# Advanced-Vision-and-Learning-Lab/sparse-view-3dgs-pack

Measured on AMD Instinct MI355X. Metric: train-step views/s (fwd+bwd) @1M Gaussians 1080p, higher is better.
Workload: dtype f32

## Files before the change

### include/gsplat.h

```cpp
#ifndef GSPLAT_H_INCLUDED
#define GSPLAT_H_INCLUDED

#include <stddef.h>
#include <stdint.h>

#ifdef __cplusplus
extern "C" {
#endif

#define GS_ABI_VERSION 7

#define GS_OK 0
#define GS_E_NULL (-1)
#define GS_E_SHAPE (-2)
#define GS_E_SCRATCH (-3)
#define GS_E_OVERFLOW (-4)
#define GS_E_UNSUPPORTED (-5)

#define GS_TILE_X 16
#define GS_TILE_Y 16
#define GS_NUM_CHANNELS 3

typedef struct GsView {
  int32_t image_height;
// ... 129 lines not shown
  void* phase1_done;
  float* extra;
  float* extra_m;
  float* extra_v;
  float* gain;
  float* gain_m;
  float* gain_v;
  float lr_extra, lr_gain;
  int32_t step_extra, step_gain;
  float* grad_out_extra;
  float* grad_out_gain;
  uint8_t* grad_mask;
  uint8_t* dormant;
  int32_t sparse;
  float* grad_out_rest;
} GsStepState;
#define GS_STEP_BLOCK 256
int gs_backward_step(const GsView* view, const GsGaussians* g, const int32_t* radii,
                     const GsScratch* scratch, int64_t num_rendered, const float* dL_dcolor,
                     const float* dL_dinvdepth, const GsStepState* st, void* workspace,
                     size_t workspace_bytes, void* stream);
int gs_backward_step_x(const GsView* view, const GsGaussians* g, const int32_t* radii,
                       const GsScratch* scratch, int64_t num_rendered, const float* dL_dcolor,
                       const float* dL_dinvdepth, const float* dL_dextra_img, const GsStepState* st,
                       void* workspace, size_t workspace_bytes, void* stream);

int gs_step_uninstanced(const GsView* view, const GsGaussians* g, const int32_t* radii,
                        const GsScratch* scratch, const GsStepState* st, void* stream);

int gs_backward_from_rows(const GsView* view, const GsGaussians* g, const int32_t* radii,
                          const GsScratch* scratch, const double* rows, int32_t depth_mode,
                          const GsGrads* grads, void* workspace, size_t workspace_bytes, void* stream);

int gs_export_tile_order(const GsScratch* scratch, int32_t W, int32_t H, uint32_t* out, void* stream);

size_t gs_tile_depth_limit_floats(int32_t W, int32_t H);
int gs_export_tile_stop_depth(const GsScratch* scratch, int32_t W, int32_t H, float* out, void* stream);
#define GS_STATUS_CHECK(tag, num_rendered, overflow, trunc_failed) \
  ((((uint32_t)(tag)) * 2654435761u) ^ (((uint32_t)(num_rendered)) * 40503u) ^ (((uint32_t)(overflow)) << 30) ^ \
   (((uint32_t)(trunc_failed)) << 31) ^ 0x5bd1e995u)
int gs_forward_status(const GsScratch* scratch, uint32_t* out , void* stream);
int gs_forward_tile_order(const GsView* view, const GsScratch* scratch, void* stream);
int gs_debug_blend_stats(const GsScratch* scratch, int32_t P, int32_t W, int32_t H, uint64_t* out, void* stream);
int gs_export_binning_region(const GsScratch* scratch, int32_t W, int32_t H, int64_t num_rendered, uint64_t* keys_sorted,
                             uint32_t* point_list, void* stream);

size_t gs_knn_tmp_bytes(int32_t P);
int gs_knn_mean_dist2(const float* xyz , int32_t P, float* out , void* tmp,
                      size_t tmp_bytes, void* stream);
int gs_knn_mean_dist2_idx(const float* xyz , int32_t P, float* out ,
                          int32_t* nearest , void* tmp, size_t tmp_bytes, void* stream);

size_t gs_grid_encode_tmp_bytes(int64_t B, int32_t D, int32_t L, int32_t C, int64_t n_slots);
int gs_grid_encode_fwd(const float* inputs, int64_t B, int32_t D, const float* embeddings, int64_t n_slots, int32_t C,
                       const int32_t* offsets, int32_t L, float S, int32_t H, int32_t gridtype, int32_t align_corners,
                       int32_t interp, float* outputs, float* dy_dx, void* stream);
int gs_grid_encode_bwd(const float* grad, const float* inputs, int64_t B, int32_t D, int64_t n_slots, int32_t C,
                       const int32_t* offsets, int32_t L, float S, int32_t H, int32_t gridtype, int32_t align_corners,
                       int32_t interp, const float* dy_dx, float* grad_embeddings, float* grad_inputs, void* tmp,
                       size_t tmp_bytes, void* stream);
int gs_sh_encode_fwd(const float* inputs, int64_t B, int32_t degree, float* outputs, void* stream);
int gs_sh_encode_bwd(const float* grad, const float* inputs, int64_t B, int32_t degree, float* grad_inputs, void* stream);


int gs_l1_fwd(const float* a, const float* b, int64_t n, float* sum, void* stream);
int gs_l1_bwd(const float* a, const float* b, int64_t n, float coef, float* grad_a,
              int32_t accumulate, void* stream);

int gs_dwt_haar_fwd(const float* x, int32_t NC, int32_t H, int32_t W, float* ll, float* lh,
                    float* hl, float* hh, void* stream);
int gs_dwt_haar_bwd(const float* dll, const float* dlh, const float* dhl, const float* dhh,
                    int32_t NC, int32_t H, int32_t W, float* dx, void* stream);

int gs_dwt2_l1_fwd(const float* pred, const float* gt, int32_t C, int32_t H, int32_t W,
                   float* band_sums, void* stream);
int gs_dwt2_l1_bwd(const float* pred, const float* gt, int32_t C, int32_t H, int32_t W,
                   const float* coef_dev, float* grad_pred, int32_t accumulate, void* stream);

int gs_elf_map(const float* img, int32_t C, int32_t H, int32_t W, float* elf_low ,
               float* elf , void* stream);
int gs_patch_means(const float* elf, int32_t H, int32_t W, int32_t patch, float* means,
                   void* stream);
int gs_patch_dwt_fwd(const float* pred, const float* gt, int32_t C, int32_t H, int32_t W,
                     int32_t patch, const uint8_t* mask, float* sums, void* stream);
int gs_patch_dwt_bwd(const float* pred, const float* gt, int32_t C, int32_t H, int32_t W,
                     int32_t patch, const uint8_t* mask, const float* coef_dev ,
                     float* grad_pred, int32_t accumulate, void* stream);

int gs_ssim_fwd(const float* img1, const float* img2, int32_t B, int32_t C, int32_t H, int32_t W,
                float C1, float C2, float* ssim_map, float* dm_dmu1, float* dm_dsigma1_sq,
                float* dm_dsigma12, void* stream);
int gs_ssim_bwd(const float* img1, const float* img2, int32_t B, int32_t C, int32_t H, int32_t W,
                float C1, float C2, const float* dL_dmap, const float* dm_dmu1,
                const float* dm_dsigma1_sq, const float* dm_dsigma12, float* dL_dimg1,
                void* stream);

int gs_l1_bwd_dev(const float* a, const float* b, int64_t n, const float* coef_dev , float* grad_a,
                  int32_t accumulate, void* stream);
int gs_l1_dwt2_fwd(const float* pred, const float* gt, int32_t C, int32_t H, int32_t W, float* l1_sum,
                   float* band_sums, void* stream);
int gs_l1_dwt2_fwd_clamp(const float* raw, const float* gt, int32_t C, int32_t H, int32_t W, float* l1_sum,
                         float* band_sums, float* clamped_out, void* stream);
int gs_l1_dwt2_patch_fwd_clamp(const float* raw, const float* gt, int32_t C, int32_t H, int32_t W, int32_t ps,
                               const uint8_t* mask, float* l1_sum, float* band_sums, float* patch_sums,
                               float* clamped_out, void* stream);
int gs_l1_dwt2_patch_bwd(const float* pred, const float* gt, int32_t C, int32_t H, int32_t W, int32_t ps,
                         const uint8_t* mask, const float* l1_coef_dev , const float* coef_dev ,
                         const float* patch_coef_dev , float* grad_pred, int32_t accumulate, void* stream);
int gs_l1_dwt2_bwd(const float* pred, const float* gt, int32_t C, int32_t H, int32_t W,
                   const float* l1_coef_dev , const float* coef_dev , float* grad_pred,
                   int32_t accumulate, void* stream);
int64_t gs_dwt_partials_count(int32_t C, int32_t H, int32_t W);
int gs_l1_dwt2_patch_fwd_clamp_p(const float* raw, const float* gt, int32_t C, int32_t H, int32_t W, int32_t ps,
                                 const uint8_t* mask, float* partials, float* clamped_out, void* stream);
int64_t gs_l1_partials_count(int64_t n);
int gs_l1_fwd_p(const float* a, const float* b, int64_t n, float* partials, void* stream);
int64_t gs_depth_l1_partials_count(int64_t n);
int gs_depth_l1(const float* invdepth, const float* mono_invdepth, const float* mask, int64_t n, float* partials, float coef,
                const float* coef_dev, float* grad, void* stream);
int gs_ssim_fwd_sum(const float* img1, const float* img2, int32_t B, int32_t C, int32_t H, int32_t W, float C1,
                    float C2, float* sum_out, float* dm_dmu1, float* dm_dsigma1_sq, float* dm_dsigma12,
                    void* stream);
int64_t gs_ssim_partials_count(int32_t B, int32_t C, int32_t H, int32_t W);
int gs_ssim_fwd_partials(const float* img1, const float* img2, int32_t B, int32_t C, int32_t H, int32_t W, float C1,
                         float C2, float* partials, float* dm_dmu1, float* dm_dsigma1_sq, float* dm_dsigma12,
                         void* stream);
int gs_ssim_bwd_uniform(const float* img1, const float* img2, int32_t B, int32_t C, int32_t H, int32_t W,
                        const float* coef_dev, const float* dm_dmu1, const float* dm_dsigma1_sq,
                        const float* dm_dsigma12, float* dL_dimg1, int32_t accumulate, const float* clamp_src,
                        void* stream);
typedef struct GsLgdwtParams {
  float lambda_dssim;
  float n_pix;
  float n_band1, n_band2;
  float dwt_w[8];
  float patch_w[3];
  float patch_weight;
  float patch_elems_per_sel;
  int32_t dwt_enable, patch_enable;
  int32_t reset_sums;
  int32_t custom_base;
  float w_l1, w_ssim;
} GsLgdwtParams;
int gs_lgdwt_combine(const float* sums, float* running_mean, const GsLgdwtParams* params , float* out,
                     void* stream);
int gs_lgdwt_combine_p(const float* sums, const float* ssim_partials, int64_t n_partials, float* running_mean,
                       const GsLgdwtParams* params , float* out, void* stream);
int gs_lgdwt_combine_pp(const float* sums, const float* ssim_partials, int64_t n_partials, const float* dwt_partials,
                        int64_t n_dwt, const float* l1_partials, int64_t n_l1, float* running_mean,
                        const GsLgdwtParams* params , float* out, void* stream);
int gs_lgdwt_fused_fwd(const float* raw, const float* gt, int32_t C, int32_t H, int32_t W, float C1, float C2, int32_t ps,
                       const uint8_t* mask, float* dwt_partials, float* ssim_partials, float* dm_dmu1, float* dm_dsigma1_sq,
                       float* dm_dsigma12, void* stream);
int gs_lgdwt_fused_bwd(const float* raw, const float* gt, int32_t C, int32_t H, int32_t W, int32_t flags, int32_t ps,
                       const uint8_t* mask, const float* coef_dev, const float* dm_dmu1, const float* dm_dsigma1_sq,
                       const float* dm_dsigma12, float* grad, void* stream);

typedef struct GsAdamSeg {
  int64_t begin, end;
  float lr_a, lr_b;
  int32_t period, split;
  int32_t step;
  int32_t row_width;
} GsAdamSeg;
int gs_adam_step(float* params, const float* grads, float* exp_avg, float* exp_avg_sq, int64_t n,
                 const GsAdamSeg* segs, int32_t nseg, float beta1, float beta2, float eps, int32_t step,
                 void* stream);
int gs_adam_step_gated(float* params, const float* grads, float* exp_avg, float* exp_avg_sq, int64_t n,
                       const GsAdamSeg* segs, int32_t nseg, float beta1, float beta2, float eps, int32_t step,
                       const float* gate, void* stream);
int gs_adam_step_masked(float* params, const float* grads, float* exp_avg, float* exp_avg_sq, int64_t n,
                        const GsAdamSeg* segs, int32_t nseg, float beta1, float beta2, float eps, int32_t step,
                        const float* gate, const float* row_mask, void* stream);

int gs_activations_fwd(const float* scaling , const float* rotation ,
                       const float* opacity , int32_t P, float* scales_out, float* rotations_out,
                       float* opacities_out, void* stream);
int gs_activations_bwd(const float* scaling, const float* rotation, const float* opacity, int32_t P,
                       const float* dL_dscales, const float* dL_drotations, const float* dL_dopacities,
                       float* d_scaling, float* d_rotation, float* d_opacity, void* stream);
int gs_densify_stats(const int32_t* radii, const float* dL_dmeans2D , int32_t P,
                     float* max_radii2D , float* xyz_gradient_accum , float* denom ,
                     void* stream);

int gs_rows_pack(const float* flat, int32_t P, int32_t nfields, const int32_t* widths , const uint8_t* mask,
                 const int32_t* pos, int32_t K, float* packed, void* stream);
int gs_rows_unpack(float* flat, int32_t P, int32_t nfields, const int32_t* widths , const uint8_t* mask,
                   const int32_t* pos, int32_t K, const float* packed, void* stream);
int64_t gs_image_stage_partials_count(int32_t H, int32_t W);
int gs_image_stage_fwd(const float* raw, const float* exposure, const float* alpha, int32_t H, int32_t W, float* pred,
                       void* stream);
int gs_image_stage_bwd(const float* raw, const float* exposure, const float* alpha, const float* g_pred, int32_t H, int32_t W,
                       float* g_raw, float* partials, void* stream);
int gs_exposure_adam(const float* partials, int64_t n_partials, int32_t camera, float* grad, float* exposure, float* exp_avg,
                     float* exp_avg_sq, int32_t n_cameras, float lr, double beta1, double beta2, float eps, int32_t step,
                     const float* gate, void* stream);
int gs_export_row_mask(const GsScratch* scratch, int32_t P, uint8_t* mask, void* stream);

int gs_profile_enable(int32_t on);
int gs_profile_only(int32_t stage);
int gs_profile_reset(void);
int gs_profile_stage_count(void);
const char* gs_profile_stage_name(int32_t stage);
int gs_profile_read(double* ms, int64_t* counts, int32_t n);

#ifdef __cplusplus
}
#endif
#endif
```

### profiles/summarize.py

```python
#!/usr/bin/env python3
import collections
import csv
import glob
import json
import os
import sys

src, tag = sys.argv[1], sys.argv[2]
script_dir = os.path.dirname(os.path.abspath(__file__))
here = sys.argv[3] if len(sys.argv) > 3 else script_dir
sys.path.insert(0, script_dir)
from source_id import source_id


def run_identity():
    ident = {"tag": tag, "source_id": source_id(os.path.dirname(script_dir))}
    try:
        line = [x for x in open(os.path.join(src, "bench_trace.json")).read().splitlines() if x.startswith("{")][-1]
        j = json.loads(line)
        ident["P"] = j["config"]["gaussians"]
        ident["R"] = j["config"]["num_rendered_last_view"]
        ident["workload"] = j["config"]["workload"]
    except Exception as e:
        ident["identity_error"] = repr(e)
    return ident
OURS = ("preprocess_fwd_kernel", "scan_block_sums_kernel", "rs_hist_kernel", "rs_scatter_kernel", "scan_reduce_kernel",
        "scan_sums_kernel", "scan_down_kernel", "rs_rowscan_kernel", "sorted_block_sums_kernel", "duplicate_kernel", "tile_ranges_kernel",
        "bin_prepare_kernel", "render_fwd_wave_kernel", "render_bwd_wave_kernel", "render_fwd_kernel", "render_bwd_kernel", "adam_kernel", "scan_small_kernel", "preprocess_bwd_kernel", "l1_fwd_kernel",
        "l1_bwd_kernel", "dwt2_l1_fwd_kernel", "dwt2_l1_bwd_kernel", "ssim_fwd_kernel", "ssim_bwd_kernel",
        "patch_dwt_kernel", "lgdwt_combine_kernel", "act_fwd_kernel", "act_bwd_kernel", "densify_stats_kernel", "patch_means_kernel", "elf_low_kernel", "bilinear_up_kernel", "knn_search_kernel", "preprocess_bwd_step_kernel",
        "tile_order_kernel", "zero_rows_kernel", "stop_depth_bounds_kernel", "region_bin_kernel", "region_prepare_kernel",
        "status_tag_kernel", "rs_small_sort_kernel", "step_uninstanced_kernel", "chain_kernel",
        "tb_entries_kernel", "tb_emit_kernel", "tb_regions_from_counts_kernel", "tb_regions_kernel", "tb_tile_count_kernel",
        "tb_region_scan_kernel", "tb_tile_scan_kernel", "tb_write_kernel", "depth_l1_kernel", "rows_pack_kernel", "row_mask_kernel",
        "ssim_fwd_clamp_kernel", "lgdwt_bwd_kernel", "lgdwt_fwd_kernel")


def short(name):
    for o in sorted(OURS, key=len, reverse=True):
        if o in name:
            return o
    return name.split("(")[0][-60:]


stats = glob.glob(os.path.join(src, "trace", "*", "*_kernel_stats.csv"))[0]
rows = list(csv.DictReader(open(stats)))
import shutil
shutil.copyfile(stats, os.path.join(here, "%s_rocprofv3_kernel_stats_full.csv" % tag))
with open(os.path.join(here, "%s_kernel_stats.csv" % tag), "w") as f:
    w = csv.writer(f)
    w.writerow(["Name", "Calls", "TotalDurationNs", "AverageNs", "Percentage", "MinNs", "MaxNs"])
    for r in rows[:40]:
        w.writerow([short(r["Name"]), r["Calls"], r["TotalDurationNs"], r["AverageNs"], r["Percentage"], r["MinNs"], r["MaxNs"]])

trace = glob.glob(os.path.join(src, "trace", "*", "*_kernel_trace.csv"))[0]
tr = sorted(csv.DictReader(open(trace)), key=lambda r: int(r["Start_Timestamp"]))
idx = [i for i, r in enumerate(tr) if "render_bwd_wave_kernel" in r["Kernel_Name"] or "render_bwd_kernel" in r["Kernel_Name"]]
a, b = idx[-3], idx[-2]
for j in range(len(idx) - 2, 0, -1):
    if any("step_uninstanced_kernel" in r["Kernel_Name"] for r in tr[idx[j - 1]:idx[j]]):
        a, b = idx[j - 1], idx[j]
        break
seg = tr[a:b]
wall = (int(tr[b]["Start_Timestamp"]) - int(seg[0]["Start_Timestamp"])) / 1e6
t_end = int(tr[b]["Start_Timestamp"])
iv = sorted((int(r["Start_Timestamp"]), min(int(r["End_Timestamp"]), t_end)) for r in seg)
busy, cur_s, cur_e = 0.0, None, None
for s0, e0 in iv:
    if cur_e is None or s0 > cur_e:
        if cur_e is not None:
            busy += cur_e - cur_s
        cur_s, cur_e = s0, e0
    else:
        cur_e = max(cur_e, e0)
busy = (busy + (cur_e - cur_s if cur_e is not None else 0)) / 1e6
agg = collections.OrderedDict()
for r in seg:
    n = short(r["Kernel_Name"])
    agg.setdefault(n, [0.0, 0])
    agg[n][0] += (int(r["End_Timestamp"]) - int(r["Start_Timestamp"])) / 1e3
    agg[n][1] += 1
with open(os.path.join(here, "%s_step_timeline.txt" % tag), "w") as f:
    f.write("one steady-state train step (render_bwd to render_bwd), rocprofv3 --kernel-trace\n")
    f.write("wall %.3f ms, GPU busy %.3f ms, %d kernel launches\n" % (wall, busy, len(seg)))
    for n, (d, c) in sorted(agg.items(), key=lambda x: -x[1][0]):
        f.write("%10.1f us %4d  %s\n" % (d, c, n))

traffic = {}
table = collections.defaultdict(lambda: {"FETCH_SIZE": [], "WRITE_SIZE": []})
for kind in ("fetch", "write"):
    files = glob.glob(os.path.join(src, kind, "*", "*_counter_collection.csv"))
    if not files:
        continue
    for r in csv.DictReader(open(files[0])):
        table[short(r["Kernel_Name"])][r["Counter_Name"]].append(float(r["Counter_Value"]))
with open(os.path.join(here, "%s_pmc_traffic.csv" % tag), "w") as f:
    w = csv.writer(f)
    w.writerow(["kernel", "launches", "FETCH_SIZE_KiB_mean", "WRITE_SIZE_KiB_mean", "hbm_read_bytes_corrected(x2)",
                "hbm_write_bytes", "hbm_total_bytes_per_launch"])
    for k, v in sorted(table.items()):
        if k not in OURS or not v["FETCH_SIZE"]:
            continue
        fs = v["FETCH_SIZE"][-max(1, len(v["FETCH_SIZE"]) // 3):]
        ws = v["WRITE_SIZE"][-max(1, len(v["WRITE_SIZE"]) // 3):] if v["WRITE_SIZE"] else [0.0]
        fm, wm = sum(fs) / len(fs), sum(ws) / len(ws)
        rd, wr = 2.0 * fm * 1024.0, wm * 1024.0
        w.writerow([k, len(v["FETCH_SIZE"]), "%.1f" % fm, "%.1f" % wm, "%.0f" % rd, "%.0f" % wr, "%.0f" % (rd + wr)])
        traffic[k] = rd + wr
stage_of = {"render_bwd": "render_bwd_wave_kernel", "render_fwd": "render_fwd_wave_kernel", "preprocess_fwd": "preprocess_fwd_kernel",
            "preprocess_bwd": "preprocess_bwd_kernel", "preprocess_bwd_step": "preprocess_bwd_step_kernel",
            "duplicate": "duplicate_kernel", "tile_ranges": "tile_ranges_kernel", "region_bin": "region_bin_kernel",
            "ssim_fwd": "ssim_fwd_kernel", "ssim_bwd": "ssim_bwd_kernel",
            "step_uninstanced": "step_uninstanced_kernel", "chain": "chain_kernel"}
for st, kn in (("ssim_fwd", "ssim_fwd_clamp_kernel"), ("ssim_fwd", "lgdwt_fwd_kernel"), ("ssim_bwd", "lgdwt_bwd_kernel")):
    if kn in traffic:
        stage_of[st] = kn
out = {st: traffic[k] for st, k in stage_of.items() if k in traffic}
out.update(run_identity())
out["launches_counted"] = {st: len(table[k]["FETCH_SIZE"]) for st, k in stage_of.items() if k in traffic}
if "region_bin_kernel" in traffic:
    out["sort"] = traffic["region_bin_kernel"]
elif "rs_scatter_kernel" in traffic:
    out["sort"] = 6 * (traffic.get("rs_scatter_kernel", 0) + traffic.get("rs_hist_kernel", 0))
json.dump(out, open(os.path.join(here, "pmc_traffic.json"), "w"), indent=1)
print(open(os.path.join(here, "%s_step_timeline.txt" % tag)).read())
print(open(os.path.join(here, "%s_pmc_traffic.csv" % tag)).read())

sq = collections.defaultdict(lambda: collections.defaultdict(list))
for f in glob.glob(os.path.join(src, "sq[0-9]*", "*", "*_counter_collection.csv")):
    for r in csv.DictReader(open(f)):
        sq[short(r["Kernel_Name"])][r["Counter_Name"]].append(float(r["Counter_Value"]))
if sq:
    with open(os.path.join(here, "%s_sq_counters.csv" % tag), "w") as f:
        w = csv.writer(f)
        w.writerow(["kernel", "waves", "VALU_insts_per_wave", "LDS_insts_per_wave", "SALU_insts_per_wave", "VMEM_rd_per_wave",
                    "VMEM_wr_per_wave", "VALU_issue_pct_of_peak", "VALU_active_x4_pct_of_SIMD_cycles", "wait_any_pct_of_wave_cycles",
                    "wait_inst_pct_of_wave_cycles", "waves_per_SIMD", "LDS_bank_conflict_pct_of_LDS_cycles"])
        sq_insts = run_identity()
        sq_insts["launches_counted"] = {}
        for k, v in sorted(sq.items()):
            m = {c: sum(x) / len(x) for c, x in v.items()}
            if k not in OURS or "GRBM_GUI_ACTIVE" not in m or m.get("SQ_WAVES", 0) == 0:
                continue
            simd_cycles = m["GRBM_GUI_ACTIVE"] / 8 * 1024
            wc = max(1.0, m.get("SQ_WAVE_CYCLES", 0))
            w.writerow([k, int(m["SQ_WAVES"]), round(m.get("SQ_INSTS_VALU", 0) / m["SQ_WAVES"], 1),
                        round(m.get("SQ_INSTS_LDS", 0) / m["SQ_WAVES"], 1), round(m.get("SQ_INSTS_SALU", 0) / m["SQ_WAVES"], 1),
                        round(m.get("SQ_INSTS_VMEM_RD", 0) / m["SQ_WAVES"], 1), round(m.get("SQ_INSTS_VMEM_WR", 0) / m["SQ_WAVES"], 1),
                        round(100 * m.get("SQ_INSTS_VALU", 0) * 2 / simd_cycles, 1),
                        round(100 * m.get("SQ_ACTIVE_INST_VALU", 0) * 4 / simd_cycles, 1),
                        round(100 * m.get("SQ_WAIT_ANY", 0) / wc, 1), round(100 * m.get("SQ_WAIT_INST_ANY", 0) / wc, 1),
                        round(wc * 4 / simd_cycles, 2),
                        round(100 * m.get("SQ_LDS_BANK_CONFLICT", 0) / max(1.0, m.get("SQ_LDS_IDX_ACTIVE", 0)), 1)])
            for st, kn in (("render_bwd", "render_bwd_wave_kernel"), ("render_fwd", "render_fwd_wave_kernel")):
                if k == kn:
                    sq_insts[st] = m.get("SQ_INSTS_VALU", 0)
                    sq_insts["launches_counted"][st] = len(v.get("SQ_INSTS_VALU", []))
                    sq_insts[st + "_valu_active_cycles_per_simd"] = m.get("SQ_ACTIVE_INST_VALU", 0) * 4 / 1024
                    sq_insts[st + "_valu_active_share_under_profiler"] = m.get("SQ_ACTIVE_INST_VALU", 0) * 4 / simd_cycles
    json.dump(sq_insts, open(os.path.join(here, "sq_insts.json"), "w"), indent=1)
    print(open(os.path.join(here, "%s_sq_counters.csv" % tag)).read())


for kind in ("init_like",):
    st_files = glob.glob(os.path.join(src, "trace_" + kind, "*", "*_kernel_stats.csv"))
    if not st_files:
        continue
    shutil.copyfile(st_files[0], os.path.join(here, "%s_%s_rocprofv3_kernel_stats_full.csv" % (tag, kind)))
    with open(os.path.join(here, "%s_%s_kernel_stats.csv" % (tag, kind)), "w") as f:
        w = csv.writer(f)
        w.writerow(["Name", "Calls", "TotalDurationNs", "AverageNs", "Percentage", "MinNs", "MaxNs"])
        for r in list(csv.DictReader(open(st_files[0])))[:30]:
            w.writerow([short(r["Name"]), r["Calls"], r["TotalDurationNs"], r["AverageNs"], r["Percentage"], r["MinNs"], r["MaxNs"]])
    ident = {"tag": tag, "source_id": source_id(os.path.dirname(script_dir)), "scene": kind}
    try:
        line = [x for x in open(os.path.join(src, "bench_trace_%s.json" % kind)).read().splitlines() if x.startswith("{")][-1]
        j = json.loads(line)
        ident["P"], ident["R"] = j["config"]["gaussians"], j["config"]["num_rendered_last_view"]
        shutil.copyfile(os.path.join(src, "bench_trace_%s.json" % kind), os.path.join(here, "%s_%s_bench_under_rocprof.json" % (tag, kind)))
    except Exception as e:
        ident["identity_error"] = repr(e)
    sqk = collections.defaultdict(lambda: collections.defaultdict(list))
    for f in glob.glob(os.path.join(src, "sq_" + kind, "*", "*_counter_collection.csv")):
        for r in csv.DictReader(open(f)):
            sqk[short(r["Kernel_Name"])][r["Counter_Name"]].append(float(r["Counter_Value"]))
    ident["launches_counted"] = {}
    for stn, kn in (("render_bwd", "render_bwd_wave_kernel"), ("render_fwd", "render_fwd_wave_kernel")):
        v = sqk.get(kn, {}).get("SQ_INSTS_VALU", [])
        if v:
            ident[stn] = sum(v) / len(v)
            ident["launches_counted"][stn] = len(v)
            wv = sqk[kn].get("SQ_WAVES", [])
            sa = sqk[kn].get("SQ_INSTS_SALU", [])
            if wv and sum(wv):
                ident[stn + "_valu_per_wave"] = sum(v) / sum(wv) * len(wv) / len(v)
                if sa:
                    ident[stn + "_salu_per_wave"] = sum(sa) / sum(wv) * len(wv) / len(sa)
    json.dump(ident, open(os.path.join(here, "sq_insts_%s.json" % kind), "w"), indent=1)
    print(kind, json.dumps(ident))


st_files = glob.glob(os.path.join(src, "trace_binning", "*", "*_kernel_stats.csv"))
if st_files:
    BIN = ("tb_", "rs_", "scan_sums_kernel", "scan_block_sums_kernel", "bin_prepare_kernel", "preprocess_fwd_kernel", "render_fwd_wave_kernel")
    with open(os.path.join(here, "%s_binning_kernel_stats.csv" % tag), "w") as f:
        w = csv.writer(f)
        w.writerow(["Name", "Calls", "TotalDurationNs", "AverageNs", "MinNs", "MaxNs"])
        for r in csv.DictReader(open(st_files[0])):
            if any(b in r["Name"] for b in BIN):
                w.writerow([r["Name"].split("(")[0][-48:], r["Calls"], r["TotalDurationNs"], r["AverageNs"], r["MinNs"], r["MaxNs"]])
    try:
        shutil.copyfile(os.path.join(src, "binning_trace.log"), os.path.join(here, "%s_binning_probe.log" % tag))
    except OSError:
        pass
    cnt = collections.defaultdict(lambda: collections.defaultdict(list))
    for d_ in ("sq_binning", "fetch_binning", "write_binning"):
        for f in glob.glob(os.path.join(src, d_, "*", "*_counter_collection.csv")):
            for r in csv.DictReader(open(f)):
                cnt[r["Kernel_Name"].split("(")[0][-48:]][r["Counter_Name"]].append(float(r["Counter_Value"]))
    with open(os.path.join(here, "%s_binning_counters.csv" % tag), "w") as f:
        w = csv.writer(f)
        w.writerow(["kernel", "launches", "hbm_read_bytes_corrected(x2)", "hbm_write_bytes", "LDS_insts_per_wave",
                    "LDS_bank_conflict_pct_of_LDS_cycles"])
        for k, v in sorted(cnt.items()):
            if not any(b in k for b in BIN):
                continue
            last = lambda x: x[-max(1, len(x) // 2):]
            m = {c: sum(last(x)) / len(last(x)) for c, x in v.items()}
            w.writerow([k, len(next(iter(v.values()))), "%.0f" % (2048.0 * m.get("FETCH_SIZE", 0)), "%.0f" % (1024.0 * m.get("WRITE_SIZE", 0)),
                        round(m.get("SQ_INSTS_LDS", 0) / max(1.0, m.get("SQ_WAVES", 0)), 1),
                        round(100 * m.get("SQ_LDS_BANK_CONFLICT", 0) / max(1.0, m.get("SQ_LDS_IDX_ACTIVE", 0)), 1)])
    print(open(os.path.join(here, "%s_binning_counters.csv" % tag)).read())
```

### sparse-view-3dgs-pack_amd/csrc/gs_loss.hip

```cpp
#include <cstdlib>

#include "gs_common.h"
#include "gs_prof.h"

#define HC 0.7071067811865476f

struct Bands {
  float ll, lh, hl, hh;
};
__device__ __forceinline__ Bands haar_block(float a, float b, float c, float d) {
  const float lo_t = HC * a + HC * b, hi_t = HC * a - HC * b;
  const float lo_b = HC * c + HC * d, hi_b = HC * c - HC * d;
  Bands r;
  r.ll = HC * lo_t + HC * lo_b;
  r.lh = HC * lo_t - HC * lo_b;
  r.hl = HC * hi_t + HC * hi_b;
  r.hh = HC * hi_t - HC * hi_b;
  return r;
}
__device__ __forceinline__ void haar_block_adj(float gll, float glh, float ghl, float ghh, float& da, float& db,
                                               float& dc, float& dd) {
  const float dlo_t = HC * gll + HC * glh, dlo_b = HC * gll - HC * glh;
  const float dhi_t = HC * ghl + HC * ghh, dhi_b = HC * ghl - HC * ghh;
  da = HC * dlo_t + HC * dhi_t;
// ... 22 lines not shown
  }
}

__global__ void __launch_bounds__(GS_BLOCK) l1_fwd_kernel(const float* __restrict__ a, const float* __restrict__ b,
                                                          int64_t n, float* sum, float* __restrict__ partials) {
  float acc[1] = {0.f};
  const int64_t n4 = n >> 2;
  const float4* a4 = reinterpret_cast<const float4*>(a);
  const float4* b4 = reinterpret_cast<const float4*>(b);
  for (int64_t i = (int64_t)blockIdx.x * GS_BLOCK + threadIdx.x; i < n4; i += (int64_t)gridDim.x * GS_BLOCK) {
    const float4 x = a4[i], y = b4[i];
    acc[0] += fabsf(x.x - y.x) + fabsf(x.y - y.y) + fabsf(x.z - y.z) + fabsf(x.w - y.w);
  }
  if (blockIdx.x == 0 && threadIdx.x < (n & 3)) acc[0] += fabsf(a[n4 * 4 + threadIdx.x] - b[n4 * 4 + threadIdx.x]);
  if (partials) {
    __shared__ float red[GS_BLOCK / 64];
    float x = acc[0];
#pragma unroll
    for (int off = 32; off >= 1; off >>= 1) x += __shfl_down(x, off, 64);
    if ((threadIdx.x & 63) == 0) red[threadIdx.x >> 6] = x;
    __syncthreads();
    if (threadIdx.x == 0) {
      float t = 0.f;
      for (int w = 0; w < GS_BLOCK / 64; w++) t += red[w];
      partials[blockIdx.x] = t;
    }
    return;
  }
  block_sum_atomic<1>(acc, sum);
}
__global__ void __launch_bounds__(GS_BLOCK) l1_bwd_kernel(const float* __restrict__ a, const float* __restrict__ b,
                                                          int64_t n, float coef, const float* __restrict__ coef_dev,
                                                          float* __restrict__ g, int accumulate) {
  if (coef_dev) coef *= coef_dev[0];
  for (int64_t i = (int64_t)blockIdx.x * GS_BLOCK + threadIdx.x; i < n; i += (int64_t)gridDim.x * GS_BLOCK) {
    const float v = coef * sgnf(a[i] - b[i]);
    g[i] = accumulate ? g[i] + v : v;
  }
}

__global__ void __launch_bounds__(GS_BLOCK) depth_l1_kernel(const float* __restrict__ d, const float* __restrict__ m,
                                                            const float* __restrict__ k, int64_t n, float* __restrict__ partials,
                                                            float coef, const float* __restrict__ coef_dev,
                                                            float* __restrict__ grad) {
  if (coef_dev) coef *= coef_dev[0];
  float acc = 0.f;
  for (int64_t i = (int64_t)blockIdx.x * GS_BLOCK + threadIdx.x; i < n; i += (int64_t)gridDim.x * GS_BLOCK) {
    const float w = k ? k[i] : 1.0f;
    const float v = (d[i] - m[i]) * w;
    acc += fabsf(v);
    if (grad) grad[i] = coef * sgnf(v) * w;
  }
  if (partials) {
    __shared__ float red[GS_BLOCK / 64];
#pragma unroll
    for (int off = 32; off >= 1; off >>= 1) acc += __shfl_down(acc, off, 64);
    if ((threadIdx.x & 63) == 0) red[threadIdx.x >> 6] = acc;
    __syncthreads();
    if (threadIdx.x == 0) {
      float t = 0.f;
      for (int w = 0; w < GS_BLOCK / 64; w++) t += red[w];
      partials[blockIdx.x] = t;
    }
  }
}

__global__ void __launch_bounds__(GS_BLOCK) dwt_fwd_kernel(const float* __restrict__ x, int NC, int H, int W, float* ll,
                                                           float* lh, float* hl, float* hh) {
  const int h = cdiv2(H), w = cdiv2(W);
  const int64_t total = (int64_t)NC * h * w;
  for (int64_t o = (int64_t)blockIdx.x * GS_BLOCK + threadIdx.x; o < total; o += (int64_t)gridDim.x * GS_BLOCK) {
    const int j = (int)(o % w), i = (int)((o / w) % h), c = (int)(o / ((int64_t)w * h));
    const float* p = x + (size_t)c * H * W;
    const int y0 = 2 * i, y1 = min(2 * i + 1, H - 1), x0 = 2 * j, x1 = min(2 * j + 1, W - 1);
    const Bands b = haar_block(p[(size_t)y0 * W + x0], p[(size_t)y0 * W + x1], p[(size_t)y1 * W + x0], p[(size_t)y1 * W + x1]);
    if (ll) ll[o] = b.ll;
    if (lh) lh[o] = b.lh;
    if (hl) hl[o] = b.hl;
    if (hh) hh[o] = b.hh;
  }
}
__global__ void __launch_bounds__(GS_BLOCK) dwt_bwd_kernel(const float* dll, const float* dlh, const float* dhl,
                                                           const float* dhh, int NC, int H, int W, float* __restrict__ dx) {
  const int h = cdiv2(H), w = cdiv2(W);
  const int64_t total = (int64_t)NC * h * w;
  for (int64_t o = (int64_t)blockIdx.x * GS_BLOCK + threadIdx.x; o < total; o += (int64_t)gridDim.x * GS_BLOCK) {
    const int j = (int)(o % w), i = (int)((o / w) % h), c = (int)(o / ((int64_t)w * h));
    float da, db, dc, dd;
    haar_block_adj(dll ? dll[o] : 0.f, dlh ? dlh[o] : 0.f, dhl ? dhl[o] : 0.f, dhh ? dhh[o] : 0.f, da, db, dc, dd);
    float* p = dx + (size_t)c * H * W;
    const int y0 = 2 * i, x0 = 2 * j;
    const bool py = 2 * i + 1 >= H, pxp = 2 * j + 1 >= W;
    if (!py && !pxp) {
      p[(size_t)y0 * W + x0] = da;
      p[(size_t)y0 * W + x0 + 1] = db;
      p[(size_t)(y0 + 1) * W + x0] = dc;
      p[(size_t)(y0 + 1) * W + x0 + 1] = dd;
    } else if (py && !pxp) {
      p[(size_t)y0 * W + x0] = da + dc;
      p[(size_t)y0 * W + x0 + 1] = db + dd;
    } else if (!py && pxp) {
      p[(size_t)y0 * W + x0] = da + db;
      p[(size_t)(y0 + 1) * W + x0] = dc + dd;
    } else {
      p[(size_t)y0 * W + x0] = ((da + db) + dc) + dd;
    }
  }
}

struct Px44 {
  float v[4][4];
};
struct Blk44 {
  float l1[2][2][4];
  float l2[4];
};
template <bool FAST>
__device__ __forceinline__ void load_px44(const float* __restrict__ p, int H, int W, int i2, int j2, int h1, int w1,
                                          Px44& o) {
  if (FAST) {
#pragma unroll
    for (int y = 0; y < 4; y++) {
      const float4 q = reinterpret_cast<const float4*>(p + (size_t)(4 * i2 + y) * W)[j2];
      o.v[y][0] = q.x; o.v[y][1] = q.y; o.v[y][2] = q.z; o.v[y][3] = q.w;
    }
  } else {
#pragma unroll
    for (int r = 0; r < 2; r++)
#pragma unroll
      for (int c = 0; c < 2; c++) {
        const int r1 = min(2 * i2 + r, h1 - 1), c1 = min(2 * j2 + c, w1 - 1);
        const int y0 = 2 * r1, y1 = min(2 * r1 + 1, H - 1), x0 = 2 * c1, x1 = min(2 * c1 + 1, W - 1);
        o.v[2 * r][2 * c] = p[(size_t)y0 * W + x0];
        o.v[2 * r][2 * c + 1] = p[(size_t)y0 * W + x1];
        o.v[2 * r + 1][2 * c] = p[(size_t)y1 * W + x0];
        o.v[2 * r + 1][2 * c + 1] = p[(size_t)y1 * W + x1];
      }
  }
}
__device__ __forceinline__ void bands_of(const Px44& x, Blk44& o) {
  float ll[2][2];
#pragma unroll
  for (int r = 0; r < 2; r++)
#pragma unroll
    for (int c = 0; c < 2; c++) {
      const Bands b = haar_block(x.v[2 * r][2 * c], x.v[2 * r][2 * c + 1], x.v[2 * r + 1][2 * c], x.v[2 * r + 1][2 * c + 1]);
      o.l1[r][c][0] = b.ll; o.l1[r][c][1] = b.lh; o.l1[r][c][2] = b.hl; o.l1[r][c][3] = b.hh;
      ll[r][c] = b.ll;
    }
  const Bands b2 = haar_block(ll[0][0], ll[0][1], ll[1][0], ll[1][1]);
  o.l2[0] = b2.ll; o.l2[1] = b2.lh; o.l2[2] = b2.hl; o.l2[3] = b2.hh;
}

template <bool FAST, bool ROWS>
__device__ __forceinline__ void dwt2_l1_fwd_body(const float* __restrict__ pred, const float* __restrict__ gt, int C, int H,
                                                 int W, float* band_sums, float* l1_sum, float* __restrict__ clamped_out,
                                                 const uint8_t* __restrict__ patch_mask, int ps, float* patch_sums,
                                                 float* __restrict__ partials, int clamp, unsigned wg, unsigned nwg,
                                                 float (*red12)[12]) {
  const int h1 = cdiv2(H), w1 = cdiv2(W), h2 = cdiv2(h1), w2 = cdiv2(w1);
  const int64_t total = (int64_t)C * h2 * w2;
  const int pnx = patch_mask ? W / ps : 0, pny = patch_mask ? H / ps : 0;
  float s[12] = {0, 0, 0, 0, 0, 0, 0, 0, 0, 0, 0, 0};
  for (int64_t o = (int64_t)wg * GS_BLOCK + threadIdx.x; o < total; o += (int64_t)nwg * GS_BLOCK) {
    const int j2 = (int)(o % w2), i2 = (int)((o / w2) % h2), c = (int)(o / ((int64_t)w2 * h2));
    Px44 pa, pb;
    load_px44<FAST>(pred + (size_t)c * H * W, H, W, i2, j2, h1, w1, pa);
    load_px44<FAST>(gt + (size_t)c * H * W, H, W, i2, j2, h1, w1, pb);
    if (FAST && (clamped_out || clamp)) {
#pragma unroll
      for (int y = 0; y < 4; y++) {
#pragma unroll
        for (int x = 0; x < 4; x++) pa.v[y][x] = fminf(fmaxf(pa.v[y][x], 0.f), 1.f);
        if (clamped_out)
          reinterpret_cast<float4*>(clamped_out + (size_t)c * H * W + (size_t)(4 * i2 + y) * W)[j2] =
              make_float4(pa.v[y][0], pa.v[y][1], pa.v[y][2], pa.v[y][3]);
      }
    }
    Blk44 a, b;
    bands_of(pa, a);
    bands_of(pb, b);
    bool in_patch = false;
    if (FAST && patch_mask) {
      const int py = (4 * i2) / ps, px = (4 * j2) / ps;
      in_patch = py < pny && px < pnx && patch_mask[py * pnx + px] != 0;
    }
#pragma unroll
    for (int r = 0; r < 2; r++)
#pragma unroll
      for (int cc = 0; cc < 2; cc++)
        if (FAST || (2 * i2 + r < h1 && 2 * j2 + cc < w1)) {
#pragma unroll
          for (int k = 0; k < 4; k++) {
            const float d = fabsf(a.l1[r][cc][k] - b.l1[r][cc][k]);
            s[k] += d;
            if (FAST && k > 0 && in_patch) s[8 + k] += d;
          }
        }
#pragma unroll
    for (int k = 0; k < 4; k++) s[4 + k] += fabsf(a.l2[k] - b.l2[k]);
    if (ROWS || l1_sum) {
#pragma unroll
      for (int y = 0; y < 4; y++)
#pragma unroll
        for (int x = 0; x < 4; x++)
          if (FAST || (4 * i2 + y < H && 4 * j2 + x < W)) s[8] += fabsf(pa.v[y][x] - pb.v[y][x]);
    }
  }
  if (ROWS || l1_sum) {
#pragma unroll
    for (int k = 0; k < 12; k++) {
      float x = s[k];
#pragma unroll
      for (int off = 32; off >= 1; off >>= 1) x += __shfl_down(x, off, 64);
      if ((threadIdx.x & 63) == 0) red12[threadIdx.x >> 6][k] = x;
    }
    __syncthreads();
    if (threadIdx.x < 12) {
      float t = 0.f;
      for (int w = 0; w < GS_BLOCK / 64; w++) t += red12[w][threadIdx.x];
      if (ROWS || partials)
        partials[(size_t)wg * 12 + threadIdx.x] = t;
      else if (t != 0.f)
        atomicAdd(threadIdx.x < 8 ? &band_sums[threadIdx.x] : (threadIdx.x == 8 ? l1_sum : &patch_sums[threadIdx.x - 9]), t);
    }
  } else {
    float s8[8];
#pragma unroll
    for (int k = 0; k < 8; k++) s8[k] = s[k];
    block_sum_atomic<8>(s8, band_sums);
  }
}
template <bool FAST>
__global__ void __launch_bounds__(GS_BLOCK) dwt2_l1_fwd_kernel(const float* __restrict__ pred, const float* __restrict__ gt,
                                                               int C, int H, int W, float* band_sums, float* l1_sum,
                                                               float* __restrict__ clamped_out,
                                                               const uint8_t* __restrict__ patch_mask, int ps,
                                                               float* patch_sums, float* __restrict__ partials, int clamp) {
  __shared__ float red12[GS_BLOCK / 64][12];
  dwt2_l1_fwd_body<FAST, false>(pred, gt, C, H, W, band_sums, l1_sum, clamped_out, patch_mask, ps, patch_sums, partials, clamp,
                         blockIdx.x, gridDim.x, red12);
}

template <bool FAST>
__global__ void __launch_bounds__(GS_BLOCK) dwt2_l1_bwd_kernel(const float* __restrict__ pred, const float* __restrict__ gt,
                                                               int C, int H, int W, const float* __restrict__ coef,
                                                               const float* __restrict__ l1_coef, float* __restrict__ grad,
                                                               int accumulate, const uint8_t* __restrict__ patch_mask, int ps,
                                                               const float* __restrict__ patch_coef) {
  const int h1 = cdiv2(H), w1 = cdiv2(W), h2 = cdiv2(h1), w2 = cdiv2(w1);
  const int64_t total = (int64_t)C * h2 * w2;
  const int pnx = patch_mask ? W / ps : 0, pny = patch_mask ? H / ps : 0;
  float cfg[8];
#pragma unroll
  for (int k = 0; k < 8; k++) cfg[k] = coef[k];
  float cp[3] = {0.f, 0.f, 0.f};
  if (patch_mask) { cp[0] = patch_coef[0]; cp[1] = patch_coef[1]; cp[2] = patch_coef[2]; }
  const float c1l = l1_coef ? l1_coef[0] : 0.f;
  for (int64_t o = (int64_t)blockIdx.x * GS_BLOCK + threadIdx.x; o < total; o += (int64_t)gridDim.x * GS_BLOCK) {
    const int j2 = (int)(o % w2), i2 = (int)((o / w2) % h2), c = (int)(o / ((int64_t)w2 * h2));
    Px44 pa, pb;
    load_px44<FAST>(pred + (size_t)c * H * W, H, W, i2, j2, h1, w1, pa);
    load_px44<FAST>(gt + (size_t)c * H * W, H, W, i2, j2, h1, w1, pb);
    Blk44 a, b;
    bands_of(pa, a);
    bands_of(pb, b);
    float cf[8];
#pragma unroll
    for (int k = 0; k < 8; k++) cf[k] = cfg[k];
    if (FAST && patch_mask) {
      const int py = (4 * i2) / ps, px = (4 * j2) / ps;
      if (py < pny && px < pnx && patch_mask[py * pnx + px] != 0) {
        cf[1] += cp[0];
        cf[2] += cp[1];
        cf[3] += cp[2];
      }
    }
    float dl[2][2];
    {
      float da, db, dc, dd;
      haar_block_adj(cf[4] * sgnf(a.l2[0] - b.l2[0]), cf[5] * sgnf(a.l2[1] - b.l2[1]), cf[6] * sgnf(a.l2[2] - b.l2[2]),
                     cf[7] * sgnf(a.l2[3] - b.l2[3]), da, db, dc, dd);
      const bool pr = !FAST && 2 * i2 + 1 >= h1, pc = !FAST && 2 * j2 + 1 >= w1;
      dl[0][0] = da; dl[0][1] = db; dl[1][0] = dc; dl[1][1] = dd;
      if (pr && pc) { dl[0][0] = ((da + db) + dc) + dd; }
      else if (pr) { dl[0][0] = da + dc; dl[0][1] = db + dd; }
      else if (pc) { dl[0][0] = da + db; dl[1][0] = dc + dd; }
    }
    float* gp = grad + (size_t)c * H * W;
    float out[4][4];
#pragma unroll
    for (int r = 0; r < 2; r++)
#pragma unroll
      for (int cc = 0; cc < 2; cc++) {
        const int r1 = 2 * i2 + r, c1 = 2 * j2 + cc;
        if (!FAST && (r1 >= h1 || c1 >= w1)) continue;
        float da, db, dc, dd;
        haar_block_adj(cf[0] * sgnf(a.l1[r][cc][0] - b.l1[r][cc][0]) + dl[r][cc], cf[1] * sgnf(a.l1[r][cc][1] - b.l1[r][cc][1]),
                       cf[2] * sgnf(a.l1[r][cc][2] - b.l1[r][cc][2]), cf[3] * sgnf(a.l1[r][cc][3] - b.l1[r][cc][3]), da, db,
                       dc, dd);
        const int y0 = 2 * r1, x0 = 2 * c1;
        const bool py = !FAST && y0 + 1 >= H, pxp = !FAST && x0 + 1 >= W;
        float v00 = da, v01 = db, v10 = dc, v11 = dd;
        if (py && pxp) v00 = ((da + db) + dc) + dd;
        else if (py) { v00 = da + dc; v01 = db + dd; }
        else if (pxp) { v00 = da + db; v10 = dc + dd; }
        v00 += c1l * sgnf(pa.v[2 * r][2 * cc] - pb.v[2 * r][2 * cc]);
        v01 += c1l * sgnf(pa.v[2 * r][2 * cc + 1] - pb.v[2 * r][2 * cc + 1]);
        v10 += c1l * sgnf(pa.v[2 * r + 1][2 * cc] - pb.v[2 * r + 1][2 * cc]);
        v11 += c1l * sgnf(pa.v[2 * r + 1][2 * cc + 1] - pb.v[2 * r + 1][2 * cc + 1]);
        if (FAST) {
          out[2 * r][2 * cc] = v00; out[2 * r][2 * cc + 1] = v01; out[2 * r + 1][2 * cc] = v10; out[2 * r + 1][2 * cc + 1] = v11;
        } else {
          float* q = gp + (size_t)y0 * W + x0;
          if (accumulate) {
            q[0] += v00;
            if (!pxp) q[1] += v01;
            if (!py) { q[W] += v10; if (!pxp) q[W + 1] += v11; }
          } else {
            q[0] = v00;
            if (!pxp) q[1] = v01;
            if (!py) { q[W] = v10; if (!pxp) q[W + 1] = v11; }
          }
        }
      }
    if (FAST) {
#pragma unroll
      for (int y = 0; y < 4; y++) {
        float4* q = reinterpret_cast<float4*>(gp + (size_t)(4 * i2 + y) * W) + j2;
        float4 v = make_float4(out[y][0], out[y][1], out[y][2], out[y][3]);
        if (accumulate) { const float4 old = *q; v.x += old.x; v.y += old.y; v.z += old.z; v.w += old.w; }
        *q = v;
      }
    }
  }
}

__global__ void __launch_bounds__(GS_BLOCK) elf_low_kernel(const float* __restrict__ img, int C, int H, int W,
                                                           float* __restrict__ low) {
  const int h = cdiv2(H), w = cdiv2(W);
  const int o = blockIdx.x * GS_BLOCK + threadIdx.x;
  if (o >= h * w) return;
  const int j = o % w, i = o / w;
  const int y0 = 2 * i, y1 = min(2 * i + 1, H - 1), x0 = 2 * j, x1 = min(2 * j + 1, W - 1);
  float s0 = 0.f, s1 = 0.f, s2 = 0.f, s3 = 0.f;
  for (int c = 0; c < C; c++) {
    const float* p = img + (size_t)c * H * W;
    const Bands b = haar_block(p[(size_t)y0 * W + x0], p[(size_t)y0 * W + x1], p[(size_t)y1 * W + x0], p[(size_t)y1 * W + x1]);
    s0 += fabsf(b.ll); s1 += fabsf(b.lh); s2 += fabsf(b.hl); s3 += fabsf(b.hh);
  }
  const float HF = s1 + s2 + s3;
  low[o] = s0 / (s0 + HF + 1e-8f);
}
__global__ void __launch_bounds__(GS_BLOCK) bilinear_up_kernel(const float* __restrict__ low, int h, int w, int H, int W,
                                                               float* __restrict__ out) {
  const int o = blockIdx.x * GS_BLOCK + threadIdx.x;
  if (o >= H * W) return;
  const int x = o % W, y = o / W;
  const float sh = (float)h / (float)H, sw = (float)w / (float)W;
  float sy = sh * ((float)y + 0.5f) - 0.5f;
  if (sy < 0) sy = 0;
  const int y0 = (int)sy, y1 = y0 + (y0 < h - 1 ? 1 : 0);
  const float ly1 = sy - (float)y0, ly0 = 1.f - ly1;
  float sx = sw * ((float)x + 0.5f) - 0.5f;
  if (sx < 0) sx = 0;
  const int x0 = (int)sx, x1 = x0 + (x0 < w - 1 ? 1 : 0);
  const float lx1 = sx - (float)x0, lx0 = 1.f - lx1;
  out[o] = ly0 * (lx0 * low[(size_t)y0 * w + x0] + lx1 * low[(size_t)y0 * w + x1]) +
           ly1 * (lx0 * low[(size_t)y1 * w + x0] + lx1 * low[(size_t)y1 * w + x1]);
}
__global__ void __launch_bounds__(GS_BLOCK) patch_means_kernel(const float* __restrict__ elf, int H, int W, int ps,
                                                               float* __restrict__ means) {
  const int nx = W / ps;
  const int px = blockIdx.x % nx, py = blockIdx.x / nx;
// ... 93 lines not shown
#pragma unroll
    for (int j = 0; j < 4; j++)
#pragma unroll
      for (int q = 0; q < NQ; q++) acc[rd][j][q] = 0.f;
    if (item < NITEM) {
      const int r = item / (ST / 4), c0 = (item % (ST / 4)) * 4;
#pragma unroll
      for (int e = 0; e < 14; e++) {
        float val[NQ];
        if (FWD) {
          const float a = tile[0][r][c0 + e], b = tile[1][r][c0 + e];
          val[0] = a; val[1] = a * a; val[2] = b; val[3 % NQ] = b * b; val[4 % NQ] = a * b;
        } else {
#pragma unroll
          for (int q = 0; q < NQ; q++) val[q] = tile[q][r][c0 + e];
        }
#pragma unroll
        for (int j = 0; j < 4; j++) {
          const int t = e - j;
          if (t >= 0 && t < 11) {
#pragma unroll
            for (int q = 0; q < NQ; q++) acc[rd][j][q] += GW[t] * val[q];
          }
        }
      }
    }
  }
  __syncthreads();
#pragma unroll
  for (int rd = 0; rd < NR; rd++) {
    const int item = threadIdx.x + rd * GS_BLOCK;
    if (item < NITEM) {
      const int r = item / (ST / 4), c0 = (item % (ST / 4)) * 4;
#pragma unroll
      for (int j = 0; j < 4; j++)
#pragma unroll
        for (int q = 0; q < NQ; q++) hor[q][r][c0 + j] = acc[rd][j][q];
    }
  }
  __syncthreads();
  const int lx = threadIdx.x & 31, r0 = (threadIdx.x >> 5) * 4;
#pragma unroll
  for (int j = 0; j < 4; j++)
#pragma unroll
    for (int q = 0; q < NQ; q++) out[j][q] = 0.f;
#pragma unroll
  for (int e = 0; e < 14; e++) {
    float val[NQ];
#pragma unroll
    for (int q = 0; q < NQ; q++) val[q] = hor[q][r0 + e][lx];
#pragma unroll
    for (int j = 0; j < 4; j++) {
      const int t = e - j;
      if (t >= 0 && t < 11) {
#pragma unroll
        for (int q = 0; q < NQ; q++) out[j][q] += GW[t] * val[q];
      }
    }
  }
}

__device__ __forceinline__ float clamp01(float v) { return fminf(fmaxf(v, 0.f), 1.f); }
__device__ __forceinline__ void ssim_stage_fwd(const float* __restrict__ img1, const float* __restrict__ img2, size_t plane,
                                               int H, int W, int bx, int by, bool clamp1, float (*tile)[SH][SH + 1]) {
  const bool vec = (W & 3) == 0 && ((((uintptr_t)img1) | ((uintptr_t)img2)) & 15) == 0;
  if (vec) {
    constexpr int VPR = 12, NV = SH * VPR, NVI = (NV + GS_BLOCK - 1) / GS_BLOCK;
    float4 a[NVI], b[NVI];
#pragma unroll
    for (int it = 0; it < NVI; it++) {
      const int v = threadIdx.x + it * GS_BLOCK;
      const int r = v / VPR, q = v % VPR;
      const int y = by + r - 5, x4 = bx - 8 + 4 * q;
      a[it] = b[it] = make_float4(0.f, 0.f, 0.f, 0.f);
      if (v < NV && y >= 0 && y < H && x4 >= 0 && x4 + 3 < W) {
        a[it] = *reinterpret_cast<const float4*>(img1 + plane + (size_t)y * W + x4);
        b[it] = *reinterpret_cast<const float4*>(img2 + plane + (size_t)y * W + x4);
      }
    }
#pragma unroll
    for (int it = 0; it < NVI; it++) {
      const int v = threadIdx.x + it * GS_BLOCK;
      if (v < NV) {
        const int r = v / VPR, c0 = 4 * (v % VPR) - 3;
        const float av[4] = {a[it].x, a[it].y, a[it].z, a[it].w}, bv[4] = {b[it].x, b[it].y, b[it].z, b[it].w};
#pragma unroll
        for (int e = 0; e < 4; e++) {
          const int c = c0 + e;
          if (c >= 0 && c < SH) {
            tile[0][r][c] = clamp1 ? clamp01(av[e]) : av[e];
            tile[1][r][c] = bv[e];
          }
        }
      }
    }
  } else {
    constexpr int NIT = (SH * SH + GS_BLOCK - 1) / GS_BLOCK;
    float a[NIT], b[NIT];
#pragma unroll
    for (int it = 0; it < NIT; it++) {
      const int k = threadIdx.x + it * GS_BLOCK;
      const int r = k / SH, c = k % SH;
      const int y = by + r - 5, x = bx + c - 5;
      a[it] = 0.f;
      b[it] = 0.f;
      if (k < SH * SH && x >= 0 && x < W && y >= 0 && y < H) {
        a[it] = img1[plane + (size_t)y * W + x];
        b[it] = img2[plane + (size_t)y * W + x];
      }
    }
#pragma unroll
    for (int it = 0; it < NIT; it++) {
      const int k = threadIdx.x + it * GS_BLOCK;
      if (k < SH * SH) {
        tile[0][k / SH][k % SH] = clamp1 ? clamp01(a[it]) : a[it];
        tile[1][k / SH][k % SH] = b[it];
      }
    }
  }
}
__device__ __forceinline__ float ssim_fwd_pixels(const float (&out)[4][5], size_t plane, int H, int W, int bx, int by, float C1,
                                                 float C2, float* __restrict__ ssim_map, float* __restrict__ dm_dmu1,
                                                 float* __restrict__ dm_dsigma1_sq, float* __restrict__ dm_dsigma12) {
  const int lx = threadIdx.x & 31, ly0 = threadIdx.x >> 5;
  float msum = 0.f;
#pragma unroll
  for (int m = 0; m < 4; m++) {
    const int x = bx + lx, y = by + 4 * ly0 + m;
    if (x >= W || y >= H) continue;
    const float mu1 = out[m][0], mu2 = out[m][2];
    const float sigma1_sq = out[m][1] - mu1 * mu1;
    const float sigma2_sq = out[m][3] - mu2 * mu2;
    const float sigma12 = out[m][4] - mu1 * mu2;
    const float mu1_sq = mu1 * mu1, mu2_sq = mu2 * mu2, mu1_mu2 = mu1 * mu2;
    const float Cc = (2.0f * mu1_mu2 + C1);
    const float D = (2.0f * sigma12 + C2);
    const float A = (mu1_sq + mu2_sq + C1);
    const float B = (sigma1_sq + sigma2_sq + C2);
    const size_t o = plane + (size_t)y * W + x;
    const float inv_AB = 1.0f / (A * B);
    const float inv_A = B * inv_AB, inv_B = A * inv_AB;
    const float mval = (Cc * D) * inv_AB;
    msum += mval;
    if (ssim_map) ssim_map[o] = mval;
    if (dm_dmu1) {
      dm_dmu1[o] = (mu2 * 2.0f * D) * inv_AB - (mu2 * 2.0f * Cc) * inv_AB - (mu1 * 2.0f * Cc * D) * inv_AB * inv_A +
                   (mu1 * 2.0f * Cc * D) * inv_AB * inv_B;
      dm_dsigma1_sq[o] = (-Cc * D) * inv_AB * inv_B;
      dm_dsigma12[o] = (2 * Cc) * inv_AB;
    }
  }
  return msum;
}
__device__ __forceinline__ void ssim_store_partial(float msum, float* __restrict__ partials, int linear) {
  __shared__ float red[GS_BLOCK / 64];
  float x = msum;
#pragma unroll
  for (int off = 32; off >= 1; off >>= 1) x += __shfl_down(x, off, 64);
  __syncthreads();
  if ((threadIdx.x & 63) == 0) red[threadIdx.x >> 6] = x;
  __syncthreads();
  if (threadIdx.x == 0)
    partials[linear] = (red[0] + red[1]) + (red[2] + red[3]);
}

__global__ void __launch_bounds__(GS_BLOCK) ssim_fwd_kernel(const float* __restrict__ img1, const float* __restrict__ img2,
                                                            int H, int W, float C1, float C2, float* __restrict__ ssim_map,
                                                            float* __restrict__ dm_dmu1, float* __restrict__ dm_dsigma1_sq,
                                                            float* __restrict__ dm_dsigma12, float* sum_out, float* __restrict__ partials,
                                                            int planes) {
  constexpr int LDS_WORDS = (2 * SH * (SH + 1) > 5 * SH * HS) ? 2 * SH * (SH + 1) : 5 * SH * HS;
  __shared__ float lds_buf[LDS_WORDS];
  float (*tile)[SH][SH + 1] = reinterpret_cast<float (*)[SH][SH + 1]>(lds_buf);
  float (*hor)[SH][HS] = reinterpret_cast<float (*)[SH][HS]>(lds_buf);
  const SsimTile tl = ssim_tile_of_block((W + ST - 1) / ST, (H + ST - 1) / ST, planes);
  if (!tl.live) return;
  const size_t plane = (size_t)tl.z * H * W;
  const int bx = tl.bx, by = tl.by;
  ssim_stage_fwd(img1, img2, plane, H, W, bx, by, false, tile);
  __syncthreads();
  float out[4][5];
  ssim_conv_tile<5, true>(tile, hor, out);
  const float msum = ssim_fwd_pixels(out, plane, H, W, bx, by, C1, C2, ssim_map, dm_dmu1, dm_dsigma1_sq, dm_dsigma12);
  if (partials) {
    ssim_store_partial(msum, partials, tl.linear);
  } else if (sum_out) {
    float acc[1] = {msum};
    __syncthreads();
    block_sum_atomic<1>(acc, sum_out);
  }
}

__device__ __forceinline__ void ssim_stage_bwd(const float* __restrict__ dL_dmap, float gu, const float* __restrict__ dm_dmu1,
                                               const float* __restrict__ dm_dsigma1_sq, const float* __restrict__ dm_dsigma12,
                                               size_t plane, int H, int W, int bx, int by, float (*tile)[SH][SH + 1]) {
  const bool vec = (W & 3) == 0 && !dL_dmap &&
                   ((((uintptr_t)dm_dmu1) | ((uintptr_t)dm_dsigma1_sq) | ((uintptr_t)dm_dsigma12)) & 15) == 0;
  if (vec) {
    constexpr int VPR = 12, NV = SH * VPR, NVI = (NV + GS_BLOCK - 1) / GS_BLOCK;
    float4 a[NVI], b[NVI], d[NVI];
#pragma unroll
    for (int it = 0; it < NVI; it++) {
      const int v = threadIdx.x + it * GS_BLOCK;
      const int r = v / VPR, q = v % VPR;
      const int y = by + r - 5, x4 = bx - 8 + 4 * q;
      a[it] = b[it] = d[it] = make_float4(0.f, 0.f, 0.f, 0.f);
      if (v < NV && y >= 0 && y < H && x4 >= 0 && x4 + 3 < W) {
        const size_t o = plane + (size_t)y * W + x4;
        a[it] = *reinterpret_cast<const float4*>(dm_dmu1 + o);
        b[it] = *reinterpret_cast<const float4*>(dm_dsigma1_sq + o);
        d[it] = *reinterpret_cast<const float4*>(dm_dsigma12 + o);
      }
    }
#pragma unroll
    for (int it = 0; it < NVI; it++) {
      const int v = threadIdx.x + it * GS_BLOCK;
      if (v < NV) {
        const int r = v / VPR, c0 = 4 * (v % VPR) - 3;
        const float av[4] = {a[it].x, a[it].y, a[it].z, a[it].w}, bv[4] = {b[it].x, b[it].y, b[it].z, b[it].w};
        const float dv[4] = {d[it].x, d[it].y, d[it].z, d[it].w};
#pragma unroll
        for (int e = 0; e < 4; e++) {
          const int c = c0 + e;
          if (c >= 0 && c < SH) {
            tile[0][r][c] = av[e] * gu;
            tile[1][r][c] = bv[e] * gu;
            tile[2][r][c] = dv[e] * gu;
          }
        }
      }
    }
  } else {
    constexpr int NIT = (SH * SH + GS_BLOCK - 1) / GS_BLOCK;
    float g[NIT], a[NIT], b[NIT], d[NIT];
#pragma unroll
    for (int it = 0; it < NIT; it++) {
      const int k = threadIdx.x + it * GS_BLOCK;
      const int r = k / SH, c = k % SH;
      const int y = by + r - 5, x = bx + c - 5;
      g[it] = a[it] = b[it] = d[it] = 0.f;
      if (k < SH * SH && x >= 0 && x < W && y >= 0 && y < H) {
        const size_t o = plane + (size_t)y * W + x;
        g[it] = dL_dmap ? dL_dmap[o] : gu;
        a[it] = dm_dmu1[o];
        b[it] = dm_dsigma1_sq[o];
        d[it] = dm_dsigma12[o];
      }
    }
#pragma unroll
    for (int it = 0; it < NIT; it++) {
      const int k = threadIdx.x + it * GS_BLOCK;
      if (k < SH * SH) {
        tile[0][k / SH][k % SH] = a[it] * g[it];
        tile[1][k / SH][k % SH] = b[it] * g[it];
        tile[2][k / SH][k % SH] = d[it] * g[it];
      }
    }
  }
}

__global__ void __launch_bounds__(GS_BLOCK) ssim_bwd_kernel(const float* __restrict__ img1, const float* __restrict__ img2,
                                                            int H, int W, const float* __restrict__ dL_dmap,
                                                            const float* __restrict__ dm_dmu1,
                                                            const float* __restrict__ dm_dsigma1_sq,
                                                            const float* __restrict__ dm_dsigma12,
                                                            float* __restrict__ dL_dimg1, const float* __restrict__ coef_dev,
                                                            int accumulate, const float* __restrict__ clamp_src, int planes) {
  constexpr int LDS_WORDS = (3 * SH * (SH + 1) > 3 * SH * HS) ? 3 * SH * (SH + 1) : 3 * SH * HS;
  __shared__ float lds_buf[LDS_WORDS];
  float (*tile)[SH][SH + 1] = reinterpret_cast<float (*)[SH][SH + 1]>(lds_buf);
  float (*hor)[SH][HS] = reinterpret_cast<float (*)[SH][HS]>(lds_buf);
  const float gu = coef_dev ? coef_dev[0] : 0.f;
  const SsimTile tl = ssim_tile_of_block((W + ST - 1) / ST, (H + ST - 1) / ST, planes);
  if (!tl.live) return;
  const size_t plane = (size_t)tl.z * H * W;
  const int bx = tl.bx, by = tl.by;
  ssim_stage_bwd(dL_dmap, gu, dm_dmu1, dm_dsigma1_sq, dm_dsigma12, plane, H, W, bx, by, tile);
  __syncthreads();
  float out[4][3];
  ssim_conv_tile<3, false>(tile, hor, out);
  const int lx = threadIdx.x & 31, ly0 = threadIdx.x >> 5;
#pragma unroll
  for (int m = 0; m < 4; m++) {
    const int x = bx + lx, y = by + 4 * ly0 + m;
    if (x >= W || y >= H) continue;
    const size_t o = plane + (size_t)y * W + x;
    const float r = clamp_src ? clamp_src[o] : 0.f;
    const float a1 = clamp_src ? (r < 0.f ? 0.f : (r > 1.f ? 1.f : r)) : img1[o];
    float dL = 0.0f;
    dL += out[m][0];
    dL += a1 * 2.0f * out[m][1];
    dL += img2[o] * out[m][2];
    if (accumulate) dL += dL_dimg1[o];
    if (clamp_src && (r < 0.f || r > 1.f)) dL = 0.f;
    dL_dimg1[o] = dL;
  }
}

#define LGDWT_CLAMP 1
#define LGDWT_DWT 2
#define LGDWT_CLAMP_MASK 4
constexpr int SSIM_FWD_LDS_WORDS = (2 * SH * (SH + 1) > 5 * SH * HS) ? 2 * SH * (SH + 1) : 5 * SH * HS;
__device__ __forceinline__ void ssim_fwd_clamp_body(const float* __restrict__ raw, const float* __restrict__ gt, int H, int W,
                                                    int planes, float C1, float C2, float* __restrict__ dm_dmu1,
                                                    float* __restrict__ dm_dsigma1_sq, float* __restrict__ dm_dsigma12,
                                                    float* __restrict__ partials, unsigned b, float* lds_buf) {
  float (*tile)[SH][SH + 1] = reinterpret_cast<float (*)[SH][SH + 1]>(lds_buf);
  float (*hor)[SH][HS] = reinterpret_cast<float (*)[SH][HS]>(lds_buf);
  const SsimTile tl = ssim_tile_of_block((W + ST - 1) / ST, (H + ST - 1) / ST, planes, b);
  if (!tl.live) return;
  const size_t plane = (size_t)tl.z * H * W;
  const int bx = tl.bx, by = tl.by;
  ssim_stage_fwd(raw, gt, plane, H, W, bx, by, true, tile);
  __syncthreads();
  float out[4][5];
  ssim_conv_tile<5, true>(tile, hor, out);
  const float msum = ssim_fwd_pixels(out, plane, H, W, bx, by, C1, C2, nullptr, dm_dmu1, dm_dsigma1_sq, dm_dsigma12);
  ssim_store_partial(msum, partials, tl.linear);
}
__global__ void __launch_bounds__(GS_BLOCK) ssim_fwd_clamp_kernel(const float* __restrict__ raw, const float* __restrict__ gt,
                                                                  int H, int W, int planes, float C1, float C2,
                                                                  float* __restrict__ dm_dmu1, float* __restrict__ dm_dsigma1_sq,
                                                                  float* __restrict__ dm_dsigma12, float* __restrict__ partials) {
  __shared__ float lds_buf[SSIM_FWD_LDS_WORDS];
  ssim_fwd_clamp_body(raw, gt, H, W, planes, C1, C2, dm_dmu1, dm_dsigma1_sq, dm_dsigma12, partials, blockIdx.x, lds_buf);
}

__global__ void __launch_bounds__(GS_BLOCK) lgdwt_fwd_kernel(const float* __restrict__ raw, const float* __restrict__ gt, int C,
                                                             int H, int W, float C1, float C2,
                                                             const uint8_t* __restrict__ patch_mask, int ps,
                                                             float* __restrict__ dwt_partials, unsigned n_dwt, unsigned dwt_every,
                                                             float* __restrict__ dm_dmu1, float* __restrict__ dm_dsigma1_sq,
                                                             float* __restrict__ dm_dsigma12, float* __restrict__ ssim_partials) {
  static_assert(SSIM_FWD_LDS_WORDS >= (GS_BLOCK / 64) * 12, "red12 lives in the SSIM tile buffer");
  __shared__ float lds_buf[SSIM_FWD_LDS_WORDS];
  const unsigned row = blockIdx.x >> 3, lane8 = blockIdx.x & 7, dwt_rows = (n_dwt + 7) >> 3;
  bool is_dwt;
  unsigned sub_row;
  if (dwt_every == 0) {
    is_dwt = row < dwt_rows;
    sub_row = is_dwt ? row : row - dwt_rows;
  } else {
    const unsigned period = row / (dwt_every + 1), q = row % (dwt_every + 1);
    if (period < dwt_rows) {
      is_dwt = q == 0;
      sub_row = is_dwt ? period : period * dwt_every + (q - 1);
    } else {
      is_dwt = false;
      sub_row = row - dwt_rows;
    }
  }
  const unsigned b = sub_row * 8 + lane8;
  if (is_dwt) {
    if (b >= n_dwt) return;
    dwt2_l1_fwd_body<true, true>(raw, gt, C, H, W, dwt_partials, dwt_partials, nullptr, patch_mask, ps, dwt_partials,
                                 dwt_partials, 1, b, n_dwt, reinterpret_cast<float (*)[12]>(lds_buf));
  } else {
    ssim_fwd_clamp_body(raw, gt, H, W, C, C1, C2, dm_dmu1, dm_dsigma1_sq, dm_dsigma12, ssim_partials, b, lds_buf);
  }
}

__device__ __forceinline__ void dwt2_l1_adjoint_col(const float (&a)[4], const float (&b)[4], int c4, const float (&cf)[8],
                                                    float c1l, float (&g)[4]) {
  float pa[4], pb[4];
#pragma unroll
  for (int m = 0; m < 4; m++) {
    pa[m] = __shfl_xor(a[m], 1, 64);
    pb[m] = __shfl_xor(b[m], 1, 64);
  }
  const bool right = (c4 & 1) != 0, cc = (c4 & 2) != 0;
  Bands A[2], B[2];
#pragma unroll
  for (int r = 0; r < 2; r++) {
    A[r] = haar_block(right ? pa[2 * r] : a[2 * r], right ? a[2 * r] : pa[2 * r], right ? pa[2 * r + 1] : a[2 * r + 1],
                      right ? a[2 * r + 1] : pa[2 * r + 1]);
    B[r] = haar_block(right ? pb[2 * r] : b[2 * r], right ? b[2 * r] : pb[2 * r], right ? pb[2 * r + 1] : b[2 * r + 1],
                      right ? b[2 * r + 1] : pb[2 * r + 1]);
  }
  float la[2][2], lb[2][2];
#pragma unroll
  for (int r = 0; r < 2; r++) {
    const float oa = __shfl_xor(A[r].ll, 2, 64), ob = __shfl_xor(B[r].ll, 2, 64);
    la[r][0] = cc ? oa : A[r].ll;
    la[r][1] = cc ? A[r].ll : oa;
    lb[r][0] = cc ? ob : B[r].ll;
    lb[r][1] = cc ? B[r].ll : ob;
  }
  const Bands a2 = haar_block(la[0][0], la[0][1], la[1][0], la[1][1]);
  const Bands b2 = haar_block(lb[0][0], lb[0][1], lb[1][0], lb[1][1]);
  float da, db, dc, dd;
  haar_block_adj(cf[4] * sgnf(a2.ll - b2.ll), cf[5] * sgnf(a2.lh - b2.lh), cf[6] * sgnf(a2.hl - b2.hl),
                 cf[7] * sgnf(a2.hh - b2.hh), da, db, dc, dd);
#pragma unroll
  for (int r = 0; r < 2; r++) {
    const float dl = r == 0 ? (cc ? db : da) : (cc ? dd : dc);
    float ea, eb, ec, ed;
    haar_block_adj(cf[0] * sgnf(A[r].ll - B[r].ll) + dl, cf[1] * sgnf(A[r].lh - B[r].lh), cf[2] * sgnf(A[r].hl - B[r].hl),
                   cf[3] * sgnf(A[r].hh - B[r].hh), ea, eb, ec, ed);
    g[2 * r] = right ? eb : ea;
    g[2 * r + 1] = right ? ed : ec;
  }
#pragma unroll
  for (int m = 0; m < 4; m++) g[m] += c1l * sgnf(a[m] - b[m]);
}

__global__ void __launch_bounds__(GS_BLOCK) __attribute__((amdgpu_waves_per_eu(7))) lgdwt_bwd_kernel(const float* __restrict__ raw, const float* __restrict__ gt, int H,
                                                             int W, int planes, int flags, const uint8_t* __restrict__ patch_mask,
                                                             int ps, const float* __restrict__ coef,
                                                             const float* __restrict__ dm_dmu1,
                                                             const float* __restrict__ dm_dsigma1_sq,
                                                             const float* __restrict__ dm_dsigma12, float* __restrict__ grad) {
  constexpr int LDS_WORDS = (3 * SH * (SH + 1) > 3 * SH * HS) ? 3 * SH * (SH + 1) : 3 * SH * HS;
  __shared__ float lds_buf[LDS_WORDS];
  float (*tile)[SH][SH + 1] = reinterpret_cast<float (*)[SH][SH + 1]>(lds_buf);
  float (*hor)[SH][HS] = reinterpret_cast<float (*)[SH][HS]>(lds_buf);
  const float gu = coef[1];
  const SsimTile tl = ssim_tile_of_block((W + ST - 1) / ST, (H + ST - 1) / ST, planes);
  if (!tl.live) return;
  const size_t plane = (size_t)tl.z * H * W;
  const int bx = tl.bx, by = tl.by;
  const int lx = threadIdx.x & 31, ly0 = threadIdx.x >> 5;
  const int x = bx + lx, y0 = by + 4 * ly0;
  const bool live = x < W && y0 < H;
  const bool clamp = (flags & LGDWT_CLAMP) != 0;
  float r[4], b[4];
#pragma unroll
  for (int m = 0; m < 4; m++) {
    const size_t o = plane + (size_t)(y0 + m) * W + x;
    r[m] = live ? raw[o] : 0.f;
    b[m] = live ? gt[o] : 0.f;
  }
  ssim_stage_bwd(nullptr, gu, dm_dmu1, dm_dsigma1_sq, dm_dsigma12, plane, H, W, bx, by, tile);
  float g[4];
  {
    float a[4];
#pragma unroll
    for (int m = 0; m < 4; m++) a[m] = clamp ? clamp01(r[m]) : r[m];
    const float c1l = coef[0];
    if ((flags & LGDWT_DWT) || patch_mask) {
      float cf[8];
#pragma unroll
      for (int k = 0; k < 8; k++) cf[k] = coef[2 + k];
      if (patch_mask) {
        const int py = y0 / ps, px = (x & ~3) / ps, pnx = W / ps, pny = H / ps;
        if (live && py < pny && px < pnx && patch_mask[py * pnx + px] != 0) {
          cf[1] += coef[10];
          cf[2] += coef[11];
          cf[3] += coef[12];
        }
      }
      dwt2_l1_adjoint_col(a, b, lx & 3, cf, c1l, g);
    } else {
#pragma unroll
      for (int m = 0; m < 4; m++) g[m] = c1l * sgnf(a[m] - b[m]);
    }
  }
  __syncthreads();
  float out[4][3];
  ssim_conv_tile<3, false>(tile, hor, out);
  if (!live) return;
#pragma unroll
  for (int m = 0; m < 4; m++) {
    const float a = clamp ? clamp01(r[m]) : r[m];
    float dL = 0.0f;
    dL += out[m][0];
    dL += a * 2.0f * out[m][1];
    dL += b[m] * out[m][2];
    dL += g[m];
    if ((flags & LGDWT_CLAMP_MASK) && (r[m] < 0.f || r[m] > 1.f)) dL = 0.f;
    grad[plane + (size_t)(y0 + m) * W + x] = dL;
  }
}

static inline int nblocks(int64_t n, int per = GS_BLOCK, int cap = 8192) {
  int64_t b = (n + per - 1) / per;
  return (int)(b < 1 ? 1 : (b > cap ? cap : b));
}

extern "C" {

int gs_l1_fwd(const float* a, const float* b, int64_t n, float* sum, void* stream) {
  if (!a || !b || !sum) return GS_E_NULL;
  if (n <= 0) return GS_OK;
  hipStream_t s = (hipStream_t)stream;
  GS_PROF(ST_L1, s);
  if ((((uintptr_t)a | (uintptr_t)b) & 15) != 0) return GS_E_UNSUPPORTED;
  hipLaunchKernelGGL(l1_fwd_kernel, dim3(nblocks(n / 4 + 1, GS_BLOCK, 512)), dim3(GS_BLOCK), 0, s, a, b, n, sum, (float*)nullptr);
  GS_LAUNCH_CHECK(s, 0);
  return GS_OK;
}
int64_t gs_l1_partials_count(int64_t n) { return n <= 0 ? 0 : (int64_t)nblocks(n / 4 + 1, GS_BLOCK, 512); }
int gs_l1_fwd_p(const float* a, const float* b, int64_t n, float* partials, void* stream) {
  if (!a || !b || !partials) return GS_E_NULL;
  if (n <= 0) return GS_OK;
  hipStream_t s = (hipStream_t)stream;
  GS_PROF(ST_L1, s);
  if ((((uintptr_t)a | (uintptr_t)b) & 15) != 0) return GS_E_UNSUPPORTED;
  hipLaunchKernelGGL(l1_fwd_kernel, dim3(nblocks(n / 4 + 1, GS_BLOCK, 512)), dim3(GS_BLOCK), 0, s, a, b, n, (float*)nullptr, partials);
  GS_LAUNCH_CHECK(s, 0);
  return GS_OK;
}
int64_t gs_depth_l1_partials_count(int64_t n) { return n <= 0 ? 0 : (int64_t)nblocks(n, 4 * GS_BLOCK, 1024); }
int gs_depth_l1(const float* invdepth, const float* mono, const float* mask, int64_t n, float* partials, float coef,
                const float* coef_dev, float* grad, void* stream) {
  if (!invdepth || !mono || (!partials && !grad)) return GS_E_NULL;
  if (n <= 0) return GS_OK;
  hipStream_t s = (hipStream_t)stream;
  GS_PROF(ST_L1, s);
  hipLaunchKernelGGL(depth_l1_kernel, dim3(nblocks(n, 4 * GS_BLOCK, 1024)), dim3(GS_BLOCK), 0, s, invdepth, mono, mask, n, partials,
                     coef, coef_dev, grad);
  GS_LAUNCH_CHECK(s, 0);
  return GS_OK;
// ... 125 lines not shown
}
int gs_l1_dwt2_patch_bwd(const float* pred, const float* gt, int32_t C, int32_t H, int32_t W, int32_t ps, const uint8_t* mask,
                         const float* l1_coef_dev, const float* coef_dev, const float* patch_coef_dev, float* grad_pred,
                         int32_t accumulate, void* stream) {
  if (!pred || !gt || !coef_dev || !l1_coef_dev || !grad_pred || !mask || !patch_coef_dev) return GS_E_NULL;
  if (C <= 0 || H <= 0 || W <= 0 || ps <= 0 || H < ps || W < ps) return GS_E_SHAPE;
  if (ps % 4 != 0) return GS_E_UNSUPPORTED;
  hipStream_t s = (hipStream_t)stream;
  GS_PROF(ST_DWT2_BWD, s);
  return dwt2_l1_bwd_launch(pred, gt, C, H, W, coef_dev, l1_coef_dev, grad_pred, accumulate, s, mask, ps, patch_coef_dev);
}
int gs_l1_dwt2_bwd(const float* pred, const float* gt, int32_t C, int32_t H, int32_t W, const float* l1_coef_dev,
                   const float* coef_dev, float* grad_pred, int32_t accumulate, void* stream) {
  if (!pred || !gt || !coef_dev || !l1_coef_dev || !grad_pred) return GS_E_NULL;
  if (C <= 0 || H <= 0 || W <= 0) return GS_E_SHAPE;
  hipStream_t s = (hipStream_t)stream;
  GS_PROF(ST_DWT2_BWD, s);
  return dwt2_l1_bwd_launch(pred, gt, C, H, W, coef_dev, l1_coef_dev, grad_pred, accumulate, s);
}
int gs_elf_map(const float* img, int32_t C, int32_t H, int32_t W, float* elf_low, float* elf, void* stream) {
  if (!img || !elf || !elf_low) return GS_E_NULL;
  if (C <= 0 || H <= 0 || W <= 0) return GS_E_SHAPE;
  hipStream_t s = (hipStream_t)stream;
  GS_PROF(ST_ELF, s);
  const int h = (H + 1) / 2, w = (W + 1) / 2;
  hipLaunchKernelGGL(elf_low_kernel, dim3((h * w + GS_BLOCK - 1) / GS_BLOCK), dim3(GS_BLOCK), 0, s, img, C, H, W, elf_low);
  hipLaunchKernelGGL(bilinear_up_kernel, dim3((H * W + GS_BLOCK - 1) / GS_BLOCK), dim3(GS_BLOCK), 0, s, elf_low, h, w, H, W, elf);
  GS_LAUNCH_CHECK(s, 0);
  return GS_OK;
}
int gs_patch_means(const float* elf, int32_t H, int32_t W, int32_t ps, float* means, void* stream) {
  if (!elf || !means) return GS_E_NULL;
  if (ps <= 0 || H < ps || W < ps) return GS_E_SHAPE;
  hipStream_t s = (hipStream_t)stream;
  GS_PROF(ST_ELF, s);
  hipLaunchKernelGGL(patch_means_kernel, dim3((H / ps) * (W / ps)), dim3(GS_BLOCK), 0, s, elf, H, W, ps, means);
  GS_LAUNCH_CHECK(s, 0);
  return GS_OK;
}
int gs_patch_dwt_fwd(const float* pred, const float* gt, int32_t C, int32_t H, int32_t W, int32_t ps, const uint8_t* mask,
                     float* sums, void* stream) {
  if (!pred || !gt || !mask || !sums) return GS_E_NULL;
  if (ps <= 0 || H < ps || W < ps || C <= 0) return GS_E_SHAPE;
  hipStream_t s = (hipStream_t)stream;
  GS_PROF(ST_PATCH, s);
  const int hp = (ps + 1) / 2;
  const int chunks = nblocks((int64_t)C * hp * hp, GS_BLOCK * 4, 64);
  hipLaunchKernelGGL(patch_dwt_kernel<false>, dim3((H / ps) * (W / ps), chunks), dim3(GS_BLOCK), 0, s, pred, gt, C, H, W, ps,
                     mask, sums, (const float*)nullptr, (float*)nullptr);
  GS_LAUNCH_CHECK(s, 0);
  return GS_OK;
}
int gs_patch_dwt_bwd(const float* pred, const float* gt, int32_t C, int32_t H, int32_t W, int32_t ps, const uint8_t* mask,
                     const float* coef_dev, float* grad_pred, int32_t accumulate, void* stream) {
  if (!pred || !gt || !mask || !coef_dev || !grad_pred) return GS_E_NULL;
  if (ps <= 0 || H < ps || W < ps || C <= 0) return GS_E_SHAPE;
  hipStream_t s = (hipStream_t)stream;
  GS_PROF(ST_PATCH, s);
  if (!accumulate) GS_HIP_CHECK(hipMemsetAsync(grad_pred, 0, sizeof(float) * (size_t)C * H * W, s));
  const int hp = (ps + 1) / 2;
  const int chunks = nblocks((int64_t)C * hp * hp, GS_BLOCK * 4, 64);
  hipLaunchKernelGGL(patch_dwt_kernel<true>, dim3((H / ps) * (W / ps), chunks), dim3(GS_BLOCK), 0, s, pred, gt, C, H, W, ps,
                     mask, (float*)nullptr, coef_dev, grad_pred);
  GS_LAUNCH_CHECK(s, 0);
  return GS_OK;
}
int gs_ssim_fwd(const float* img1, const float* img2, int32_t B, int32_t C, int32_t H, int32_t W, float C1, float C2,
                float* ssim_map, float* dm_dmu1, float* dm_dsigma1_sq, float* dm_dsigma12, void* stream) {
  if (!img1 || !img2 || !ssim_map) return GS_E_NULL;
  if (dm_dmu1 && (!dm_dsigma1_sq || !dm_dsigma12)) return GS_E_NULL;
  if (B <= 0 || C <= 0 || H <= 0 || W <= 0 || (int64_t)B * C > 65535) return GS_E_SHAPE;
  hipStream_t s = (hipStream_t)stream;
  GS_PROF(ST_SSIM_FWD, s);
  hipLaunchKernelGGL(ssim_fwd_kernel, dim3(ssim_launch_blocks(W, H, B * C)), dim3(GS_BLOCK), 0, s, img1, img2, H, W,
                     C1, C2, ssim_map, dm_dmu1, dm_dsigma1_sq, dm_dsigma12, (float*)nullptr, (float*)nullptr, B * C);
  GS_LAUNCH_CHECK(s, 0);
  return GS_OK;
}
int gs_ssim_bwd(const float* img1, const float* img2, int32_t B, int32_t C, int32_t H, int32_t W, float, float,
                const float* dL_dmap, const float* dm_dmu1, const float* dm_dsigma1_sq, const float* dm_dsigma12,
                float* dL_dimg1, void* stream) {
  if (!img1 || !img2 || !dL_dmap || !dm_dmu1 || !dm_dsigma1_sq || !dm_dsigma12 || !dL_dimg1) return GS_E_NULL;
  if (B <= 0 || C <= 0 || H <= 0 || W <= 0 || (int64_t)B * C > 65535) return GS_E_SHAPE;
  hipStream_t s = (hipStream_t)stream;
  GS_PROF(ST_SSIM_BWD, s);
  hipLaunchKernelGGL(ssim_bwd_kernel, dim3(ssim_launch_blocks(W, H, B * C)), dim3(GS_BLOCK), 0, s, img1, img2, H, W,
                     dL_dmap, dm_dmu1, dm_dsigma1_sq, dm_dsigma12, dL_dimg1, (const float*)nullptr, 0, (const float*)nullptr, B * C);
  GS_LAUNCH_CHECK(s, 0);
  return GS_OK;
}


int gs_l1_bwd_dev(const float* a, const float* b, int64_t n, const float* coef_dev, float* grad_a, int32_t accumulate,
                  void* stream) {
  if (!a || !b || !grad_a || !coef_dev) return GS_E_NULL;
  if (n <= 0) return GS_OK;
  hipStream_t s = (hipStream_t)stream;
  GS_PROF(ST_L1, s);
  hipLaunchKernelGGL(l1_bwd_kernel, dim3(nblocks(n)), dim3(GS_BLOCK), 0, s, a, b, n, 1.0f, coef_dev, grad_a, accumulate);
  GS_LAUNCH_CHECK(s, 0);
  return GS_OK;
}

int gs_ssim_fwd_sum(const float* img1, const float* img2, int32_t B, int32_t C, int32_t H, int32_t W, float C1, float C2,
                    float* sum_out, float* dm_dmu1, float* dm_dsigma1_sq, float* dm_dsigma12, void* stream) {
  if (!img1 || !img2 || !sum_out) return GS_E_NULL;
  if (dm_dmu1 && (!dm_dsigma1_sq || !dm_dsigma12)) return GS_E_NULL;
  if (B <= 0 || C <= 0 || H <= 0 || W <= 0 || (int64_t)B * C > 65535) return GS_E_SHAPE;
  hipStream_t s = (hipStream_t)stream;
  GS_PROF(ST_SSIM_FWD, s);
  hipLaunchKernelGGL(ssim_fwd_kernel, dim3(ssim_launch_blocks(W, H, B * C)), dim3(GS_BLOCK), 0, s, img1, img2, H, W,
                     C1, C2, (float*)nullptr, dm_dmu1, dm_dsigma1_sq, dm_dsigma12, sum_out, (float*)nullptr, B * C);
  GS_LAUNCH_CHECK(s, 0);
  return GS_OK;
}

int64_t gs_ssim_partials_count(int32_t B, int32_t C, int32_t H, int32_t W) {
  if (B <= 0 || C <= 0 || H <= 0 || W <= 0) return 0;
  return (int64_t)((W + ST - 1) / ST) * ((H + ST - 1) / ST) * B * C;
}

int gs_ssim_fwd_partials(const float* img1, const float* img2, int32_t B, int32_t C, int32_t H, int32_t W, float C1, float C2,
                         float* partials, float* dm_dmu1, float* dm_dsigma1_sq, float* dm_dsigma12, void* stream) {
  if (!img1 || !img2 || !partials) return GS_E_NULL;
  if (dm_dmu1 && (!dm_dsigma1_sq || !dm_dsigma12)) return GS_E_NULL;
  if (B <= 0 || C <= 0 || H <= 0 || W <= 0 || (int64_t)B * C > 65535) return GS_E_SHAPE;
  hipStream_t s = (hipStream_t)stream;
  GS_PROF(ST_SSIM_FWD, s);
  hipLaunchKernelGGL(ssim_fwd_kernel, dim3(ssim_launch_blocks(W, H, B * C)), dim3(GS_BLOCK), 0, s, img1, img2, H, W,
                     C1, C2, (float*)nullptr, dm_dmu1, dm_dsigma1_sq, dm_dsigma12, (float*)nullptr, partials, B * C);
  GS_LAUNCH_CHECK(s, 0);
  return GS_OK;
}

int gs_ssim_bwd_uniform(const float* img1, const float* img2, int32_t B, int32_t C, int32_t H, int32_t W,
                        const float* coef_dev, const float* dm_dmu1, const float* dm_dsigma1_sq, const float* dm_dsigma12,
                        float* dL_dimg1, int32_t accumulate, const float* clamp_src, void* stream) {
  if (!img1 || !img2 || !coef_dev || !dm_dmu1 || !dm_dsigma1_sq || !dm_dsigma12 || !dL_dimg1) return GS_E_NULL;
  if (B <= 0 || C <= 0 || H <= 0 || W <= 0 || (int64_t)B * C > 65535) return GS_E_SHAPE;
  hipStream_t s = (hipStream_t)stream;
  GS_PROF(ST_SSIM_BWD, s);
  hipLaunchKernelGGL(ssim_bwd_kernel, dim3(ssim_launch_blocks(W, H, B * C)), dim3(GS_BLOCK), 0, s, img1, img2, H, W,
                     (const float*)nullptr, dm_dmu1, dm_dsigma1_sq, dm_dsigma12, dL_dimg1, coef_dev, accumulate, clamp_src, B * C);
  GS_LAUNCH_CHECK(s, 0);
  return GS_OK;
}

__global__ void __launch_bounds__(1024) lgdwt_combine_kernel(const float* __restrict__ sums_in, float* running_mean,
                                                             GsLgdwtParams p, float* __restrict__ out,
                                                             const float* __restrict__ ssim_partials, int n_partials,
                                                             const float* __restrict__ dwt_partials, int n_dwt,
                                                             const float* __restrict__ l1_partials, int n_l1) {
  __shared__ float s_extra[13];
  {
    const int slot = threadIdx.x >> 6, lane = threadIdx.x & 63;
    if (slot < 13) {
      float t = 0.f;
      if (slot < 12) {
        for (int w = lane; w < n_dwt; w += 64) t += dwt_partials[(size_t)w * 12 + slot];
      } else {
        for (int w = lane; w < n_l1; w += 64) t += l1_partials[w];
      }
#pragma unroll
      for (int off = 32; off >= 1; off >>= 1) t += __shfl_down(t, off, 64);
      if (lane == 0) s_extra[slot] = t;
    }
  }
  __syncthreads();
  float sums[16];
#pragma unroll
  for (int k = 0; k < 16; k++) sums[k] = 0.f;
  if (threadIdx.x == 0) {
#pragma unroll
    for (int k = 0; k < 16; k++) sums[k] = sums_in[k];
    sums[0] += s_extra[8] + s_extra[12];
#pragma unroll
    for (int k = 0; k < 8; k++) sums[2 + k] += s_extra[k];
#pragma unroll
    for (int k = 0; k < 3; k++) sums[10 + k] += s_extra[9 + k];
  }
  __shared__ float red[16];
  float part = 0.f;
  for (int i = threadIdx.x; i < n_partials; i += 1024) part += ssim_partials[i];
#pragma unroll
  for (int off = 32; off >= 1; off >>= 1) part += __shfl_down(part, off, 64);
  if ((threadIdx.x & 63) == 0) red[threadIdx.x >> 6] = part;
  __syncthreads();
  if (threadIdx.x != 0) return;
  const float l1 = sums[0] / p.n_pix;
  float ptot = 0.f;
  for (int w = 0; w < 16; w++) ptot += red[w];
  const float ssim = (sums[1] + ptot) / p.n_pix;
  const float w_l1 = p.custom_base ? p.w_l1 : 1.0f - p.lambda_dssim, w_ssim = p.custom_base ? p.w_ssim : p.lambda_dssim;
  const float base = w_l1 * l1 + w_ssim * (1.0f - ssim);
  float loss = base;
  float dwt = 0.f, scale = 0.f, patch = 0.f;
  for (int k = 0; k < 24; k++) out[k] = 0.f;
  out[7] = running_mean[0];
  if (p.dwt_enable) {
    for (int k = 0; k < 8; k++) {
      const float cnt = k < 4 ? p.n_band1 : p.n_band2;
      dwt += p.dwt_w[k] * (sums[2 + k] / cnt);
    }
    const float ratio = base / (dwt + 1e-8f);
    const float m = 0.95f * running_mean[0] + 0.05f * ratio;
    running_mean[0] = m;
    scale = fminf(fmaxf(m, 0.1f), 10.0f);
    loss = base + scale * dwt;
    for (int k = 0; k < 8; k++) out[10 + k] = scale * p.dwt_w[k] / (k < 4 ? p.n_band1 : p.n_band2);
  }
  if (p.patch_enable) {
    const float denom = fmaxf(sums[13] * p.patch_elems_per_sel, 1.0f);
    for (int k = 0; k < 3; k++) {
      patch += p.patch_w[k] * (sums[10 + k] / denom);
      out[18 + k] = p.patch_weight * p.patch_w[k] / denom;
    }
    loss = loss + p.patch_weight * patch;
  }
  out[0] = loss; out[1] = base; out[2] = dwt; out[3] = patch; out[4] = scale; out[5] = l1; out[6] = ssim;
  out[8] = w_l1 / p.n_pix;
  out[9] = -w_ssim / p.n_pix;
  if (p.reset_sums) {
    float* z = const_cast<float*>(sums_in);
    for (int k = 0; k < 13; k++) z[k] = 0.f;
  }
}

int gs_lgdwt_combine_pp(const float* sums, const float* ssim_partials, int64_t n_partials, const float* dwt_partials,
                        int64_t n_dwt, const float* l1_partials, int64_t n_l1, float* running_mean, const GsLgdwtParams* p,
                        float* out, void* stream) {
  if (!sums || !running_mean || !p || !out) return GS_E_NULL;
  if (n_partials < 0 || n_partials > 0x7FFFFFFF || (n_partials > 0 && !ssim_partials)) return GS_E_SHAPE;
  if (n_dwt < 0 || n_dwt > 65536 || (n_dwt > 0 && !dwt_partials) || n_l1 < 0 || n_l1 > 65536 || (n_l1 > 0 && !l1_partials))
    return GS_E_SHAPE;
  hipStream_t s = (hipStream_t)stream;
  (void)hipGetLastError();
  hipLaunchKernelGGL(lgdwt_combine_kernel, dim3(1), dim3(1024), 0, s, sums, running_mean, *p, out, ssim_partials,
                     (int)n_partials, dwt_partials, (int)n_dwt, l1_partials, (int)n_l1);
  GS_LAUNCH_CHECK(s, 0);
  return GS_OK;
}
int gs_lgdwt_combine_p(const float* sums, const float* ssim_partials, int64_t n_partials, float* running_mean,
                       const GsLgdwtParams* p, float* out, void* stream) {
  return gs_lgdwt_combine_pp(sums, ssim_partials, n_partials, nullptr, 0, nullptr, 0, running_mean, p, out, stream);
}
int gs_lgdwt_combine(const float* sums, float* running_mean, const GsLgdwtParams* p, float* out, void* stream) {
  return gs_lgdwt_combine_p(sums, nullptr, 0, running_mean, p, out, stream);
}

static inline bool lgdwt_fused_ok(const void* a, const void* b, const void* c, const void* d, const void* e, int32_t C, int32_t H,
                                  int32_t W) {
  return (H % 4) == 0 && (W % 4) == 0 && C <= 65535 &&
         ((((uintptr_t)a | (uintptr_t)b | (uintptr_t)c | (uintptr_t)d | (uintptr_t)e) & 15) == 0);
}
static inline int lgdwt_fused_args(int32_t C, int32_t H, int32_t W, int32_t ps, const uint8_t* mask) {
  if (C <= 0 || H <= 0 || W <= 0 || ps < 0) return GS_E_SHAPE;
  if ((ps > 0) != (mask != nullptr)) return GS_E_NULL;
  if (ps > 0 && (H < ps || W < ps)) return GS_E_SHAPE;
  if (ps % 4 != 0) return GS_E_UNSUPPORTED;
  return GS_OK;
}
int gs_lgdwt_fused_fwd(const float* raw, const float* gt, int32_t C, int32_t H, int32_t W, float C1, float C2, int32_t ps,
                       const uint8_t* mask, float* dwt_partials, float* ssim_partials, float* dm_dmu1, float* dm_dsigma1_sq,
                       float* dm_dsigma12, void* stream) {
  if (!raw || !gt || !dwt_partials || !ssim_partials || !dm_dmu1 || !dm_dsigma1_sq || !dm_dsigma12) return GS_E_NULL;
  const int rc = lgdwt_fused_args(C, H, W, ps, mask);
  if (rc != GS_OK) return rc;
  if (!lgdwt_fused_ok(raw, gt, dm_dmu1, dm_dsigma1_sq, dm_dsigma12, C, H, W)) return GS_E_UNSUPPORTED;
  hipStream_t s = (hipStream_t)stream;
  static const bool split = [] { const char* e = getenv("GS_LGDWT_FWD_SPLIT"); return e && atoi(e) != 0; }();
  if (split) {
    {
      GS_PROF(ST_DWT2_FWD, s);
      float dummy_target = 0.f;
      const int r = dwt2_l1_fwd_launch(raw, gt, C, H, W, &dummy_target, &dummy_target, s, nullptr, mask, ps, &dummy_target,
                                       dwt_partials, true);
      if (r != GS_OK) return r;
    }
    GS_PROF(ST_SSIM_FWD, s);
    hipLaunchKernelGGL(ssim_fwd_clamp_kernel, dim3(ssim_launch_blocks(W, H, C)), dim3(GS_BLOCK), 0, s, raw, gt, H, W, C, C1, C2,
                       dm_dmu1, dm_dsigma1_sq, dm_dsigma12, ssim_partials);
    GS_LAUNCH_CHECK(s, 0);
    return GS_OK;
  }
  const unsigned n_ssim = ssim_launch_blocks(W, H, C), n_dwt = dwt2_fwd_workgroups(C, H, W);
  const unsigned ssim_rows = n_ssim / 8, dwt_rows = (n_dwt + 7) / 8;
  const unsigned every = ssim_rows / dwt_rows < 4 ? ssim_rows / dwt_rows : 4;
  GS_PROF(ST_SSIM_FWD, s);
  hipLaunchKernelGGL(lgdwt_fwd_kernel, dim3((ssim_rows + dwt_rows) * 8), dim3(GS_BLOCK), 0, s, raw, gt, C, H, W, C1, C2, mask, ps,
                     dwt_partials, n_dwt, every, dm_dmu1, dm_dsigma1_sq, dm_dsigma12, ssim_partials);
  GS_LAUNCH_CHECK(s, 0);
  return GS_OK;
}
int gs_lgdwt_fused_bwd(const float* raw, const float* gt, int32_t C, int32_t H, int32_t W, int32_t flags, int32_t ps,
                       const uint8_t* mask, const float* coef_dev, const float* dm_dmu1, const float* dm_dsigma1_sq,
                       const float* dm_dsigma12, float* grad, void* stream) {
  if (!raw || !gt || !coef_dev || !dm_dmu1 || !dm_dsigma1_sq || !dm_dsigma12 || !grad) return GS_E_NULL;
  const int rc = lgdwt_fused_args(C, H, W, ps, mask);
  if (rc != GS_OK) return rc;
  if (!lgdwt_fused_ok(raw, gt, dm_dmu1, dm_dsigma1_sq, dm_dsigma12, C, H, W) || ((uintptr_t)grad & 15) != 0)
    return GS_E_UNSUPPORTED;
  hipStream_t s = (hipStream_t)stream;
  GS_PROF(ST_SSIM_BWD, s);
  hipLaunchKernelGGL(lgdwt_bwd_kernel, dim3(ssim_launch_blocks(W, H, C)), dim3(GS_BLOCK), 0, s, raw, gt, H, W, C, flags, mask, ps,
                     coef_dev, dm_dmu1, dm_dsigma1_sq, dm_dsigma12, grad);
  GS_LAUNCH_CHECK(s, 0);
  return GS_OK;
}
}
```

### sparse-view-3dgs-pack_amd/gsplat_amd/capi.py

```python
import ctypes as C
import os

c_f_p = C.c_void_p


class GsView(C.Structure):
    _fields_ = [
        ("image_height", C.c_int32),
        ("image_width", C.c_int32),
        ("tanfovx", C.c_float),
        ("tanfovy", C.c_float),
        ("scale_modifier", C.c_float),
        ("sh_degree", C.c_int32),
        ("prefiltered", C.c_int32),
        ("antialiasing", C.c_int32),
        ("debug", C.c_int32),
        ("tile_cull", C.c_int32),
        ("bg", C.c_void_p),
        ("viewmatrix", C.c_void_p),
        ("projmatrix", C.c_void_p),
        ("campos", C.c_void_p),
    ]


# ... 9 lines not shown
        ("rotations", C.c_void_p),
        ("cov3D_precomp", C.c_void_p),
        ("extra_channel", C.c_void_p),
        ("raw_activations", C.c_int32),
        ("extra_gain", C.c_void_p),
        ("shs_rest", C.c_void_p),
    ]


class GsScratch(C.Structure):
    _fields_ = [
        ("geom", C.c_void_p),
        ("geom_bytes", C.c_size_t),
        ("img", C.c_void_p),
        ("img_bytes", C.c_size_t),
        ("binning", C.c_void_p),
        ("binning_bytes", C.c_size_t),
        ("binning_capacity", C.c_int64),
        ("tile_order_hint", C.c_void_p),
        ("tile_depth_limit", C.c_void_p),
        ("tile_order_out", C.c_void_p),
        ("tile_depth_limit_out", C.c_void_p),
        ("binned", C.c_int32),
        ("defer_tile_order", C.c_int32),
        ("step_tag", C.c_void_p),
        ("tile_depth_limit_slack", C.c_void_p),
        ("status_host", C.c_void_p),
    ]


class GsGrads(C.Structure):
    _fields_ = [
        ("dL_dmeans3D", C.c_void_p),
        ("dL_dmeans2D", C.c_void_p),
        ("dL_dsh", C.c_void_p),
        ("dL_dcolors", C.c_void_p),
        ("dL_dopacity", C.c_void_p),
        ("dL_dscales", C.c_void_p),
        ("dL_drotations", C.c_void_p),
        ("dL_dcov3D", C.c_void_p),
        ("dL_dextra", C.c_void_p),
    ]


class GsLgdwtParams(C.Structure):
    _fields_ = [("lambda_dssim", C.c_float), ("n_pix", C.c_float), ("n_band1", C.c_float), ("n_band2", C.c_float),
                ("dwt_w", C.c_float * 8), ("patch_w", C.c_float * 3), ("patch_weight", C.c_float),
                ("patch_elems_per_sel", C.c_float), ("dwt_enable", C.c_int32), ("patch_enable", C.c_int32),
                ("reset_sums", C.c_int32), ("custom_base", C.c_int32), ("w_l1", C.c_float), ("w_ssim", C.c_float)]


class GsAdamSeg(C.Structure):
    _fields_ = [("begin", C.c_int64), ("end", C.c_int64), ("lr_a", C.c_float), ("lr_b", C.c_float),
                ("period", C.c_int32), ("split", C.c_int32), ("step", C.c_int32), ("row_width", C.c_int32)]


class GsStepState(C.Structure):
    _fields_ = [("xyz", C.c_void_p), ("features", C.c_void_p), ("opacity", C.c_void_p), ("scaling", C.c_void_p),
                ("rotation", C.c_void_p), ("m", C.c_void_p * 5), ("v", C.c_void_p * 5), ("lr", C.c_float * 6),
                ("step", C.c_int32 * 5), ("beta1", C.c_float), ("beta2", C.c_float), ("eps", C.c_float),
                ("max_radii2D", C.c_void_p), ("xyz_gradient_accum", C.c_void_p), ("denom", C.c_void_p),
                ("coef_dev", C.c_void_p), ("rows_override", C.c_void_p), ("grad_out", C.c_void_p * 5),
                ("fail_flag", C.c_void_p), ("phase", C.c_int32), ("rows_clean", C.c_int32),
                ("phase1_done", C.c_void_p),
                ("extra", C.c_void_p), ("extra_m", C.c_void_p), ("extra_v", C.c_void_p), ("gain", C.c_void_p),
                ("gain_m", C.c_void_p), ("gain_v", C.c_void_p), ("lr_extra", C.c_float), ("lr_gain", C.c_float),
                ("step_extra", C.c_int32), ("step_gain", C.c_int32), ("grad_out_extra", C.c_void_p),
                ("grad_out_gain", C.c_void_p), ("grad_mask", C.c_void_p), ("dormant", C.c_void_p), ("sparse", C.c_int32),
                ("grad_out_rest", C.c_void_p)]


_P = C.c_void_p
_I32 = C.c_int32
_I64 = C.c_int64
_F = C.c_float
_SZ = C.c_size_t

PROTOTYPES = {
    "abi_version": (C.c_int, []),
    "struct_bytes": (C.c_size_t, [C.c_int32]),
    "build_info": (C.c_char_p, []),
    "scratch_bytes": (C.c_int, [_I32, _I32, _I32, _I64, C.POINTER(_SZ), C.POINTER(_SZ)]),
    "forward_geometry": (C.c_int, [C.POINTER(GsView), C.POINTER(GsGaussians), C.POINTER(GsScratch), _P, _P, _P]),
    "forward_render": (C.c_int, [C.POINTER(GsView), C.POINTER(GsGaussians), C.POINTER(GsScratch), _P, _P, _P]),
    "backward": (C.c_int, [C.POINTER(GsView), C.POINTER(GsGaussians), _P, C.POINTER(GsScratch), _I64, _P, _P,
                           C.POINTER(GsGrads), _P, _SZ, _P]),
    "forward_render_x": (C.c_int, [C.POINTER(GsView), C.POINTER(GsGaussians), C.POINTER(GsScratch), _P, _P, _P, _P]),
    "backward_x": (C.c_int, [C.POINTER(GsView), C.POINTER(GsGaussians), _P, C.POINTER(GsScratch), _I64, _P, _P, _P,
                             C.POINTER(GsGrads), _P, _SZ, _P]),
    "forward_render_fsgs": (C.c_int, [C.POINTER(GsView), C.POINTER(GsGaussians), C.POINTER(GsScratch), _P, _P, _P, _P]),
    "backward_fsgs": (C.c_int, [C.POINTER(GsView), C.POINTER(GsGaussians), _P, C.POINTER(GsScratch), _I64, _P, _P, _P,
                                C.POINTER(GsGrads), _P, _SZ, _P]),
    "step_uninstanced": (C.c_int, [C.POINTER(GsView), C.POINTER(GsGaussians), _P, C.POINTER(GsScratch),
                                   C.POINTER(GsStepState), _P]),
    "backward_step": (C.c_int, [C.POINTER(GsView), C.POINTER(GsGaussians), _P, C.POINTER(GsScratch), _I64, _P, _P,
                                C.POINTER(GsStepState), _P, _SZ, _P]),
    "backward_step_x": (C.c_int, [C.POINTER(GsView), C.POINTER(GsGaussians), _P, C.POINTER(GsScratch), _I64, _P, _P, _P,
                                  C.POINTER(GsStepState), _P, _SZ, _P]),
    "backward_from_rows": (C.c_int, [C.POINTER(GsView), C.POINTER(GsGaussians), _P, C.POINTER(GsScratch), _P, _I32,
                                     C.POINTER(GsGrads), _P, _SZ, _P]),
    "mark_visible": (C.c_int, [_I32, _P, _P, _P, _P, _P]),
    "export_geom": (C.c_int, [C.POINTER(GsScratch), _I32, _P, _P, _P, _P, _P, _P, _P, _P, _P]),
    "export_binning": (C.c_int, [C.POINTER(GsScratch), _I64, _P, _P, _P]),
    "export_img": (C.c_int, [C.POINTER(GsScratch), _I32, _I32, _P, _P, _P, _P]),
    "export_tile_order": (C.c_int, [C.POINTER(GsScratch), _I32, _I32, _P, _P]),
    "export_tile_stop_depth": (C.c_int, [C.POINTER(GsScratch), _I32, _I32, _P, _P]),
    "forward_status": (C.c_int, [C.POINTER(GsScratch), _P, _P]),
    "forward_tile_order": (C.c_int, [C.POINTER(GsView), C.POINTER(GsScratch), _P]),
    "forward_bin": (C.c_int, [C.POINTER(GsView), C.POINTER(GsGaussians), C.POINTER(GsScratch), _P, _P]),
    "export_binning_region": (C.c_int, [C.POINTER(GsScratch), _I32, _I32, _I64, _P, _P, _P]),
    "debug_blend_stats": (C.c_int, [C.POINTER(GsScratch), _I32, _I32, _I32, _P, _P]),
    "tile_depth_limit_floats": (C.c_size_t, [_I32, _I32]),
    "knn_tmp_bytes": (_SZ, [_I32]),
    "knn_mean_dist2": (C.c_int, [_P, _I32, _P, _P, _SZ, _P]),
    "knn_mean_dist2_idx": (C.c_int, [_P, _I32, _P, _P, _P, _SZ, _P]),
    "grid_encode_tmp_bytes": (_SZ, [_I64, _I32, _I32, _I32, _I64]),
    "grid_encode_fwd": (C.c_int, [_P, _I64, _I32, _P, _I64, _I32, _P, _I32, _F, _I32, _I32, _I32, _I32, _P, _P, _P]),
    "grid_encode_bwd": (C.c_int, [_P, _P, _I64, _I32, _I64, _I32, _P, _I32, _F, _I32, _I32, _I32, _I32, _P, _P, _P, _P,
                                  _SZ, _P]),
    "sh_encode_fwd": (C.c_int, [_P, _I64, _I32, _P, _P]),
    "sh_encode_bwd": (C.c_int, [_P, _P, _I64, _I32, _P, _P]),
    "l1_fwd": (C.c_int, [_P, _P, _I64, _P, _P]),
    "l1_bwd": (C.c_int, [_P, _P, _I64, _F, _P, _I32, _P]),
    "dwt_haar_fwd": (C.c_int, [_P, _I32, _I32, _I32, _P, _P, _P, _P, _P]),
    "dwt_haar_bwd": (C.c_int, [_P, _P, _P, _P, _I32, _I32, _I32, _P, _P]),
    "dwt2_l1_fwd": (C.c_int, [_P, _P, _I32, _I32, _I32, _P, _P]),
    "dwt2_l1_bwd": (C.c_int, [_P, _P, _I32, _I32, _I32, _P, _P, _I32, _P]),
    "elf_map": (C.c_int, [_P, _I32, _I32, _I32, _P, _P, _P]),
    "patch_means": (C.c_int, [_P, _I32, _I32, _I32, _P, _P]),
    "patch_dwt_fwd": (C.c_int, [_P, _P, _I32, _I32, _I32, _I32, _P, _P, _P]),
    "patch_dwt_bwd": (C.c_int, [_P, _P, _I32, _I32, _I32, _I32, _P, _P, _P, _I32, _P]),
    "ssim_fwd": (C.c_int, [_P, _P, _I32, _I32, _I32, _I32, _F, _F, _P, _P, _P, _P, _P]),
    "ssim_bwd": (C.c_int, [_P, _P, _I32, _I32, _I32, _I32, _F, _F, _P, _P, _P, _P, _P, _P]),
    "dwt_partials_count": (C.c_int64, [_I32, _I32, _I32]),
    "l1_dwt2_patch_fwd_clamp_p": (C.c_int, [_P, _P, _I32, _I32, _I32, _I32, _P, _P, _P, _P]),
    "l1_partials_count": (C.c_int64, [_I64]),
    "l1_fwd_p": (C.c_int, [_P, _P, _I64, _P, _P]),
    "depth_l1_partials_count": (C.c_int64, [_I64]),
    "depth_l1": (C.c_int, [_P, _P, _P, _I64, _P, _F, _P, _P, _P]),
    "lgdwt_combine_pp": (C.c_int, [_P, _P, _I64, _P, _I64, _P, _I64, _P, C.POINTER(GsLgdwtParams), _P, _P]),
    "l1_bwd_dev": (C.c_int, [_P, _P, _I64, _P, _P, _I32, _P]),
    "l1_dwt2_fwd": (C.c_int, [_P, _P, _I32, _I32, _I32, _P, _P, _P]),
    "l1_dwt2_fwd_clamp": (C.c_int, [_P, _P, _I32, _I32, _I32, _P, _P, _P, _P]),
    "l1_dwt2_patch_fwd_clamp": (C.c_int, [_P, _P, _I32, _I32, _I32, _I32, _P, _P, _P, _P, _P, _P]),
    "l1_dwt2_patch_bwd": (C.c_int, [_P, _P, _I32, _I32, _I32, _I32, _P, _P, _P, _P, _P, _I32, _P]),
    "l1_dwt2_bwd": (C.c_int, [_P, _P, _I32, _I32, _I32, _P, _P, _P, _I32, _P]),
    "ssim_fwd_sum": (C.c_int, [_P, _P, _I32, _I32, _I32, _I32, _F, _F, _P, _P, _P, _P, _P]),
    "ssim_bwd_uniform": (C.c_int, [_P, _P, _I32, _I32, _I32, _I32, _P, _P, _P, _P, _P, _I32, _P, _P]),
    "lgdwt_combine": (C.c_int, [_P, _P, C.POINTER(GsLgdwtParams), _P, _P]),
    "lgdwt_combine_p": (C.c_int, [_P, _P, _I64, _P, C.POINTER(GsLgdwtParams), _P, _P]),
    "ssim_partials_count": (C.c_int64, [_I32, _I32, _I32, _I32]),
    "ssim_fwd_partials": (C.c_int, [_P, _P, _I32, _I32, _I32, _I32, _F, _F, _P, _P, _P, _P, _P]),
    "lgdwt_fused_fwd": (C.c_int, [_P, _P, _I32, _I32, _I32, _F, _F, _I32, _P, _P, _P, _P, _P, _P, _P]),
    "lgdwt_fused_bwd": (C.c_int, [_P, _P, _I32, _I32, _I32, _I32, _I32, _P, _P, _P, _P, _P, _P, _P]),
    "adam_step": (C.c_int, [_P, _P, _P, _P, _I64, C.POINTER(GsAdamSeg), _I32, _F, _F, _F, _I32, _P]),
    "adam_step_gated": (C.c_int, [_P, _P, _P, _P, _I64, C.POINTER(GsAdamSeg), _I32, _F, _F, _F, _I32, _P, _P]),
    "adam_step_masked": (C.c_int, [_P, _P, _P, _P, _I64, C.POINTER(GsAdamSeg), _I32, _F, _F, _F, _I32, _P, _P, _P]),
    "activations_fwd": (C.c_int, [_P, _P, _P, _I32, _P, _P, _P, _P]),
    "activations_bwd": (C.c_int, [_P, _P, _P, _I32, _P, _P, _P, _P, _P, _P, _P]),
    "densify_stats": (C.c_int, [_P, _P, _I32, _P, _P, _P, _P]),
    "profile_enable": (C.c_int, [_I32]),
    "profile_only": (C.c_int, [_I32]),
    "profile_reset": (C.c_int, []),
    "profile_stage_count": (C.c_int, []),
    "rows_pack": (C.c_int, [_P, _I32, _I32, C.POINTER(C.c_int32), _P, _P, _I32, _P, _P]),
    "rows_unpack": (C.c_int, [_P, _I32, _I32, C.POINTER(C.c_int32), _P, _P, _I32, _P, _P]),
    "export_row_mask": (C.c_int, [C.POINTER(GsScratch), _I32, _P, _P]),
    "profile_stage_name": (C.c_char_p, [_I32]),
    "profile_read": (C.c_int, [C.POINTER(C.c_double), C.POINTER(_I64), _I32]),
    "image_stage_partials_count": (C.c_int64, [_I32, _I32]),
    "image_stage_fwd": (C.c_int, [_P, _P, _P, _I32, _I32, _P, _P]),
    "image_stage_bwd": (C.c_int, [_P, _P, _P, _P, _I32, _I32, _P, _P, _P]),
    "exposure_adam": (C.c_int, [_P, _I64, _I32, _P, _P, _P, _P, _I32, _F, C.c_double, C.c_double, _F, _I32, _P, _P]),
}

DEVICE_ONLY = ("export_row_mask", "backward_step", "backward_step_x", "step_uninstanced", "export_tile_order", "export_tile_stop_depth", "forward_status", "forward_bin", "export_binning_region", "debug_blend_stats", "adam_step_gated", "tile_depth_limit_floats", "profile_enable", "profile_only", "profile_reset", "profile_stage_count", "profile_stage_name", "profile_read",
               "forward_render_x", "backward_x", "forward_tile_order",
               "image_stage_partials_count", "image_stage_fwd", "image_stage_bwd", "exposure_adam",
               "lgdwt_fused_fwd", "lgdwt_fused_bwd",
               "grid_encode_tmp_bytes", "grid_encode_fwd", "grid_encode_bwd", "sh_encode_fwd", "sh_encode_bwd")

ERRORS = {-1: "GS_E_NULL", -2: "GS_E_SHAPE", -3: "GS_E_SCRATCH", -4: "GS_E_OVERFLOW", -5: "GS_E_UNSUPPORTED"}


class GsError(RuntimeError):
    def __init__(self, fn, code):
        self.code = code
        what = ERRORS.get(code, "hipError_t %d" % code if code > 0 else "error %d" % code)
        super().__init__("%s failed: %s" % (fn, what))


class CApi:

    def __init__(self, path, prefix="gs_", optional=()):
        if not os.path.exists(path):
            raise ImportError(
                "gsplat native library not found at %s - build it first (python __graft_entry__.py "
                "or `make -C sparse-view-3dgs-pack_amd/csrc`); there is no fallback path." % path)
        self.path = path
        self.prefix = prefix
        self.lib = C.CDLL(path)
        self.missing = []
        for name, (res, args) in PROTOTYPES.items():
            try:
                f = getattr(self.lib, prefix + name)
            except AttributeError:
                if name in optional:
                    self.missing.append(name)
                    continue
                raise ImportError("%s does not export %s%s" % (path, prefix, name))
            f.restype = res
            f.argtypes = args
            setattr(self, "_" + name, f)

    def call(self, name, *args):
        rc = getattr(self, "_" + name)(*args)
        if rc != 0:
            raise GsError(self.prefix + name, rc)

    def raw(self, name):
        return getattr(self, "_" + name)


def read_profile(api):
    n = api.raw("profile_stage_count")()
    ms = (C.c_double * n)()
    cnt = (C.c_int64 * n)()
    api.call("profile_read", ms, cnt, n)
    return {api.raw("profile_stage_name")(i).decode(): (ms[i], cnt[i]) for i in range(n) if cnt[i] > 0}
```

### sparse-view-3dgs-pack_amd/gsplat_amd/losses.py

```python
import ctypes as C

import torch

BANDS = ("LL1", "LH1", "HL1", "HH1", "LL2", "LH2", "HL2", "HH2")

FUSED_PASSES = True


def _stream(t):
    return C.c_void_p(torch.cuda.current_stream(t.device).cuda_stream) if t.is_cuda else None


def _c(t):
    t = t.contiguous()
    return t if t.dtype == torch.float32 else t.float()


def _p(t):
    return None if t is None else t.data_ptr()


class LossOps:
    def __init__(self, api):
        self.api = api
        self._unit = {}
        ops = self

        class _L1(torch.autograd.Function):
            @staticmethod
            def forward(ctx, a, b):
                a, b = _c(a), _c(b)
                s = torch.zeros((1,), dtype=torch.float32, device=a.device)
                ops.api.call("l1_fwd", a.data_ptr(), b.data_ptr(), a.numel(), s.data_ptr(), _stream(a))
                ctx.save_for_backward(a, b)
                return (s / a.numel()).reshape(())

            @staticmethod
            def backward(ctx, g):
                a, b = ctx.saved_tensors
                coef = (g / a.numel()).reshape(1).contiguous()
                ga = torch.empty_like(a)
                if hasattr(ops.api, "_l1_bwd_dev"):
                    ops.api.call("l1_bwd_dev", a.data_ptr(), b.data_ptr(), a.numel(), coef.data_ptr(), ga.data_ptr(), 0, _stream(a))
                else:
                    ops.api.call("l1_bwd", a.data_ptr(), b.data_ptr(), a.numel(), 1.0, ga.data_ptr(), 0, _stream(a))
                    ga = ga * coef
                return ga, (-ga if ctx.needs_input_grad[1] else None)

        class _Haar(torch.autograd.Function):
            @staticmethod
            def forward(ctx, x):
                x = _c(x)
                N, Cc, H, W = x.shape
                h, w = (H + 1) // 2, (W + 1) // 2
                outs = [torch.empty((N, Cc, h, w), dtype=torch.float32, device=x.device) for _ in range(4)]
                ops.api.call("dwt_haar_fwd", x.data_ptr(), N * Cc, H, W, *[o.data_ptr() for o in outs], _stream(x))
                ctx.shape = (N, Cc, H, W)
                return tuple(outs)

            @staticmethod
            def backward(ctx, dll, dlh, dhl, dhh):
                N, Cc, H, W = ctx.shape
                gs = [None if g is None else _c(g) for g in (dll, dlh, dhl, dhh)]
                ref = next(g for g in gs if g is not None)
                dx = torch.empty((N, Cc, H, W), dtype=torch.float32, device=ref.device)
                ops.api.call("dwt_haar_bwd", *[_p(g) for g in gs], N * Cc, H, W, dx.data_ptr(), _stream(ref))
                return dx

        class _Dwt2L1(torch.autograd.Function):

            @staticmethod
            def forward(ctx, pred, gt, weights):
                pred, gt = _c(pred), _c(gt)
                Cc, H, W = pred.shape[-3:]
                sums = torch.zeros((8,), dtype=torch.float32, device=pred.device)
                ops.api.call("dwt2_l1_fwd", pred.data_ptr(), gt.data_ptr(), Cc, H, W, sums.data_ptr(), _stream(pred))
                h1, w1 = (H + 1) // 2, (W + 1) // 2
                h2, w2 = (h1 + 1) // 2, (w1 + 1) // 2
                counts = torch.tensor([Cc * h1 * w1] * 4 + [Cc * h2 * w2] * 4, dtype=torch.float32, device=pred.device)
                wdev = weights.to(device=pred.device, dtype=torch.float32)
                means = sums / counts
                ctx.save_for_backward(pred, gt, wdev / counts)
                ctx.mark_non_differentiable(means)
                return (means * wdev).sum(), means

            @staticmethod
            def backward(ctx, g, _gm):
                pred, gt, coef = ctx.saved_tensors
                coef = (coef * g).contiguous()
                Cc, H, W = pred.shape[-3:]
                grad = torch.empty_like(pred)
                ops.api.call("dwt2_l1_bwd", pred.data_ptr(), gt.data_ptr(), Cc, H, W, coef.data_ptr(), grad.data_ptr(),
                             0, _stream(pred))
                return grad, None, None

        class _PatchDwt(torch.autograd.Function):
            @staticmethod
            def forward(ctx, pred, gt, mask, ps, w3):
                pred, gt = _c(pred), _c(gt)
                Cc, H, W = pred.shape[-3:]
                sums = torch.zeros((3,), dtype=torch.float32, device=pred.device)
                ops.api.call("patch_dwt_fwd", pred.data_ptr(), gt.data_ptr(), Cc, H, W, ps, mask.data_ptr(),
                             sums.data_ptr(), _stream(pred))
                hp = (ps + 1) // 2
                n_sel = mask.sum().to(torch.float32)
                denom = torch.clamp_min(n_sel * (Cc * hp * hp), 1.0)
                w3 = w3.to(device=pred.device, dtype=torch.float32)
                ctx.save_for_backward(pred, gt, mask, w3 / denom)
                ctx.ps = ps
                return (sums / denom * w3).sum()

            @staticmethod
            def backward(ctx, g):
                pred, gt, mask, coef = ctx.saved_tensors
                coef = (coef * g).contiguous()
                Cc, H, W = pred.shape[-3:]
                grad = torch.empty_like(pred)
                ops.api.call("patch_dwt_bwd", pred.data_ptr(), gt.data_ptr(), Cc, H, W, ctx.ps, mask.data_ptr(),
                             coef.data_ptr(), grad.data_ptr(), 0, _stream(pred))
                return grad, None, None, None, None

        class _SSIMMap(torch.autograd.Function):
            @staticmethod
            def forward(ctx, C1, C2, img1, img2, padding="same", train=True):
                img1, img2 = _c(img1), _c(img2)
                B, Cc, H, W = img1.shape
                smap = torch.empty_like(img1)
                if train:
                    d1, d2, d3 = torch.empty_like(img1), torch.empty_like(img1), torch.empty_like(img1)
                else:
                    d1 = d2 = d3 = None
                ops.api.call("ssim_fwd", img1.data_ptr(), img2.data_ptr(), B, Cc, H, W, float(C1), float(C2),
                             smap.data_ptr(), _p(d1), _p(d2), _p(d3), _stream(img1))
                if padding == "valid":
                    smap = smap[:, :, 5:-5, 5:-5]
                if train:
                    ctx.save_for_backward(img1.detach(), img2, d1, d2, d3)
                ctx.C1, ctx.C2, ctx.padding, ctx.train = C1, C2, padding, train
                return smap

            @staticmethod
            def backward(ctx, opt_grad):
                if not ctx.train:
                    raise RuntimeError("fused_ssim(train=False) cannot be differentiated")
                img1, img2, d1, d2, d3 = ctx.saved_tensors
                dL_dmap = opt_grad
                if ctx.padding == "valid":
                    dL_dmap = torch.zeros_like(img1)
                    dL_dmap[:, :, 5:-5, 5:-5] = opt_grad
                dL_dmap = _c(dL_dmap)
                B, Cc, H, W = img1.shape
                grad = torch.empty_like(img1)
                ops.api.call("ssim_bwd", img1.data_ptr(), img2.data_ptr(), B, Cc, H, W, float(ctx.C1), float(ctx.C2),
                             dL_dmap.data_ptr(), d1.data_ptr(), d2.data_ptr(), d3.data_ptr(), grad.data_ptr(),
                             _stream(img1))
                return None, None, grad, None, None, None

        class _DepthL1(torch.autograd.Function):

            @staticmethod
            def forward(ctx, invdepth, mono, mask):
                d, m = _c(invdepth), _c(mono)
                k = None if mask is None else _c(mask)
                n = d.numel()
                part = torch.empty((int(ops.api.raw("depth_l1_partials_count")(n)),), dtype=torch.float32, device=d.device)
                ops.api.call("depth_l1", d.data_ptr(), m.data_ptr(), _p(k), n, part.data_ptr(), 0.0, None, None, _stream(d))
                ctx.save_for_backward(d, m, k)
                return (part.sum() / n).reshape(())

            @staticmethod
            def backward(ctx, g):
                d, m, k = ctx.saved_tensors
                coef = g.reshape(1).to(torch.float32).contiguous()
                grad = torch.empty_like(d)
                ops.api.call("depth_l1", d.data_ptr(), m.data_ptr(), _p(k), d.numel(), None, 1.0 / d.numel(), coef.data_ptr(),
                             grad.data_ptr(), _stream(d))
                return grad, None, None

        self._L1, self._Haar, self._Dwt2L1, self._PatchDwt, self._SSIMMap = _L1, _Haar, _Dwt2L1, _PatchDwt, _SSIMMap
        self._DepthL1 = _DepthL1

    def unit_grad(self, device):
        device = torch.device(device)
        u = self._unit.get(device)
        if u is None:
            u = self._unit[device] = torch.ones((), dtype=torch.float32, device=device)
        return u

    def l1_loss(self, network_output, gt):
        return self._L1.apply(network_output, gt)

    def depth_l1(self, invdepth, mono_invdepth, depth_mask=None):
        return self._DepthL1.apply(invdepth, mono_invdepth, depth_mask)

    def depth_l1_step(self, invdepth, mono_invdepth, depth_mask, weight):
        d, m = _c(invdepth), _c(mono_invdepth)
        k = None if depth_mask is None else _c(depth_mask)
        n = d.numel()
        part = torch.empty((int(self.api.raw("depth_l1_partials_count")(n)),), dtype=torch.float32, device=d.device)
        grad = torch.empty_like(d)
        self.api.call("depth_l1", d.data_ptr(), m.data_ptr(), _p(k), n, part.data_ptr(), float(weight) / n, None, grad.data_ptr(),
                      _stream(d))
        return part.sum() * (float(weight) / n), grad

    def fused_ssim(self, img1, img2, padding="same", train=True):
        assert padding in ("same", "valid")
        return self._SSIMMap.apply(0.01 ** 2, 0.03 ** 2, img1, img2, padding, train).mean()

    def ssim(self, img1, img2, window_size=11, size_average=True):
        if window_size != 11:
            raise NotImplementedError("only the 11-tap window of the reference is implemented")
        a = img1 if img1.dim() == 4 else img1.unsqueeze(0)
        b = img2 if img2.dim() == 4 else img2.unsqueeze(0)
        m = self._SSIMMap.apply(0.01 ** 2, 0.03 ** 2, a, b, "same", True)
        return m.mean() if size_average else m.mean(1).mean(1).mean(1)

    def dwt_haar(self, x):
        return self._Haar.apply(x)

    def get_dwt_subbands(self, x):
        LL1, LH1, HL1, HH1 = self.dwt_haar(x)
        LL2, LH2, HL2, HH2 = self.dwt_haar(LL1)
        return {"LL1": LL1, "LH1": LH1, "HL1": HL1, "HH1": HH1, "LL2": LL2, "LH2": LH2, "HL2": HL2, "HH2": HH2}

    def dwt_l1_loss(self, pred, gt, weights):
        w = torch.as_tensor(weights, dtype=torch.float32)
        if pred.dim() == 4:
            assert pred.shape[0] == 1, "batch of one image, as in the reference training loop"
            pred, gt = pred[0], gt[0]
        return self._Dwt2L1.apply(pred, gt, w)

    def compute_elf_map(self, image):
        image = _c(image)
        N, Cc, H, W = image.shape
        out = torch.empty((N, 1, H, W), dtype=torch.float32, device=image.device)
        low = torch.empty(((H + 1) // 2, (W + 1) // 2), dtype=torch.float32, device=image.device)
        for n in range(N):
            self.api.call("elf_map", image[n].data_ptr(), Cc, H, W, low.data_ptr(), out[n].data_ptr(), _stream(image))
        return out

    def patch_mask(self, elf_map, patch_size=128, percentile=0.2):
        elf_map = _c(elf_map)
        H, W = elf_map.shape[-2:]
        L = (H // patch_size) * (W // patch_size)
        means = torch.empty((L,), dtype=torch.float32, device=elf_map.device)
        self.api.call("patch_means", elf_map.data_ptr(), H, W, patch_size, means.data_ptr(), _stream(elf_map))
        k = int(means.numel() * (1.0 - percentile))
        k = max(1, k)
        k = min(k, means.numel())
        threshold, _ = torch.kthvalue(means, k)
        return (means >= threshold).to(torch.uint8), means

    def compute_patch_dwt_loss(self, pred, gt, elf_map, patch_size=128, percentile=0.2, lh1_weight=1.0,
                               hl1_weight=1.0, mask=None):
        N, Cc, H, W = pred.shape
        if H < patch_size or W < patch_size:
            return torch.tensor(0.0, device=pred.device)
        assert N == 1, "batch of one image, as in the reference training loop"
        if mask is None:
            mask, _ = self.patch_mask(elf_map, patch_size, percentile)
        w3 = torch.tensor([lh1_weight, hl1_weight, 0.5 * (lh1_weight + hl1_weight)], dtype=torch.float32)
        return self._PatchDwt.apply(pred[0], gt[0], mask, int(patch_size), w3)


class FusedLGDWTLoss(torch.autograd.Function):

    @staticmethod
    def forward(ctx, ops, raw, gt, mask, sums, running_mean, params, stage=None):
        api = ops.api
        raw, gt = _c(raw), _c(gt)
        Cc, H, W = raw.shape
        st = _stream(raw)
        if stage is not None:
            stage.raw = raw
            raw = torch.empty_like(raw)
            api.call("image_stage_fwd", stage.raw.data_ptr(), _p(stage.exposure), _p(stage.alpha), H, W, raw.data_ptr(), st)
        d1, d2, d3 = torch.empty_like(raw), torch.empty_like(raw), torch.empty_like(raw)
        patch_folded = bool(params.patch_enable and params.dwt_enable and H % 4 == 0 and W % 4 == 0
                            and ctx_ps(params) % 4 == 0)
        dwt_part = l1_part = None
        fast = H % 4 == 0 and W % 4 == 0
        fused = bool(FUSED_PASSES and params.fused_shape and hasattr(api, "_lgdwt_fused_bwd")
                     and (patch_folded or not params.patch_enable) and raw.data_ptr() % 16 == 0 and gt.data_ptr() % 16 == 0)
        ctx.fused = fused
        ctx.fused_flags = ((1 if params.clamp or patch_folded else 0) | (2 if params.dwt_enable else 0)
                           | (4 if params.clamp and stage is None else 0))
        partials = torch.empty((params.n_ssim_partials,), dtype=torch.float32, device=raw.device)
        if fused and (patch_folded or (params.dwt_enable and params.clamp)):
            img = None
            dwt_part = torch.empty((params.n_dwt_partials * 12,), dtype=torch.float32, device=raw.device)
            api.call("lgdwt_fused_fwd", raw.data_ptr(), gt.data_ptr(), Cc, H, W, 0.01 ** 2, 0.03 ** 2,
                     ctx_ps(params) if patch_folded else 0, mask.data_ptr() if patch_folded else None, dwt_part.data_ptr(),
                     partials.data_ptr(), d1.data_ptr(), d2.data_ptr(), d3.data_ptr(), st)
        elif patch_folded or (params.dwt_enable and fast and params.clamp):
            img = torch.empty_like(raw)
            dwt_part = torch.empty((params.n_dwt_partials * 12,), dtype=torch.float32, device=raw.device)
            api.call("l1_dwt2_patch_fwd_clamp_p", raw.data_ptr(), gt.data_ptr(), Cc, H, W, ctx_ps(params) if patch_folded else 0,
                     mask.data_ptr() if patch_folded else None, dwt_part.data_ptr(), img.data_ptr(), st)
        elif params.dwt_enable:
            img = raw.clamp(0, 1) if params.clamp else raw
            api.call("l1_dwt2_fwd", img.data_ptr(), gt.data_ptr(), Cc, H, W, sums.data_ptr(), sums[2:].data_ptr(), st)
        else:
            img = raw.clamp(0, 1) if params.clamp else raw
            if img.numel() % 4 == 0:
                l1_part = torch.empty((params.n_l1_partials,), dtype=torch.float32, device=raw.device)
                api.call("l1_fwd_p", img.data_ptr(), gt.data_ptr(), img.numel(), l1_part.data_ptr(), st)
            else:
                api.call("l1_fwd", img.data_ptr(), gt.data_ptr(), img.numel(), sums.data_ptr(), st)
        if img is not None:
            api.call("ssim_fwd_partials", img.data_ptr(), gt.data_ptr(), 1, Cc, H, W, 0.01 ** 2, 0.03 ** 2,
                     partials.data_ptr(), d1.data_ptr(), d2.data_ptr(), d3.data_ptr(), st)
        if params.patch_enable and not patch_folded:
            api.call("patch_dwt_fwd", img.data_ptr(), gt.data_ptr(), Cc, H, W, ctx_ps(params), mask.data_ptr(),
                     sums[10:].data_ptr(), st)
        out = torch.empty((24,), dtype=torch.float32, device=raw.device)
        api.call("lgdwt_combine_pp", sums.data_ptr(), partials.data_ptr(), partials.numel(),
                 None if dwt_part is None else dwt_part.data_ptr(), 0 if dwt_part is None else dwt_part.numel() // 12,
                 None if l1_part is None else l1_part.data_ptr(), 0 if l1_part is None else l1_part.numel(),
                 running_mean.data_ptr(), C.byref(params.c), out.data_ptr(), st)
        ctx.ops, ctx.params, ctx.patch_folded, ctx.stage = ops, params, patch_folded, stage
        ctx.save_for_backward(raw, img, gt, mask, d1, d2, d3, out)
        ctx.mark_non_differentiable(out)
        ctx.set_materialize_grads(False)
        return out[0], out

    @staticmethod
    def backward(ctx, g, _gout):
        raw, img, gt, mask, d1, d2, d3, out = ctx.saved_tensors
        if g is None:
            return (None,) * 8
        api, params = ctx.ops.api, ctx.params
        Cc, H, W = raw.shape
        st = _stream(raw)
        unit = ctx.ops._unit.get(g.device)
        coef = out[8:24] if (unit is not None and g.data_ptr() == unit.data_ptr()) else (out[8:24] * g).contiguous()
        grad = torch.empty_like(raw)
        if getattr(ctx, "fused", False):
            hook = getattr(ctx.ops, "before_last_backward_kernel", None)
            if hook is not None:
                hook()
            ps = ctx_ps(params) if params.patch_enable else 0
            api.call("lgdwt_fused_bwd", raw.data_ptr(), gt.data_ptr(), Cc, H, W, ctx.fused_flags, ps,
                     mask.data_ptr() if ps else None, coef.data_ptr(), d1.data_ptr(), d2.data_ptr(), d3.data_ptr(),
                     grad.data_ptr(), st)
            return None, _image_stage_bwd(api, getattr(ctx, "stage", None), grad, H, W, st), None, None, None, None, None, None
        if ctx.patch_folded:
            api.call("l1_dwt2_patch_bwd", img.data_ptr(), gt.data_ptr(), Cc, H, W, ctx_ps(params), mask.data_ptr(),
                     coef.data_ptr(), coef[2:].data_ptr(), coef[10:].data_ptr(), grad.data_ptr(), 0, st)
        elif params.dwt_enable:
            api.call("l1_dwt2_bwd", img.data_ptr(), gt.data_ptr(), Cc, H, W, coef.data_ptr(), coef[2:].data_ptr(),
                     grad.data_ptr(), 0, st)
        else:
            api.call("l1_bwd_dev", img.data_ptr(), gt.data_ptr(), img.numel(), coef.data_ptr(), grad.data_ptr(), 0, st)
        if params.patch_enable and not ctx.patch_folded:
            api.call("patch_dwt_bwd", img.data_ptr(), gt.data_ptr(), Cc, H, W, ctx_ps(params), mask.data_ptr(),
                     coef[10:].data_ptr(), grad.data_ptr(), 1, st)
        hook = getattr(ctx.ops, "before_last_backward_kernel", None)
        if hook is not None:
            hook()
        stage = getattr(ctx, "stage", None)
        api.call("ssim_bwd_uniform", img.data_ptr(), gt.data_ptr(), 1, Cc, H, W, coef[1:].data_ptr(), d1.data_ptr(),
                 d2.data_ptr(), d3.data_ptr(), grad.data_ptr(), 1,
                 raw.data_ptr() if params.clamp and stage is None else None, st)
        return None, _image_stage_bwd(api, stage, grad, H, W, st), None, None, None, None, None, None


def _image_stage_bwd(api, stage, grad, H, W, st):
    if stage is None:
        return grad
    g_raw = torch.empty_like(grad)
    api.call("image_stage_bwd", stage.raw.data_ptr(), _p(stage.exposure), _p(stage.alpha), grad.data_ptr(), H, W,
             g_raw.data_ptr(), _p(stage.partials), st)
    if stage.exposure_grad is not None:
        api.call("exposure_adam", stage.partials.data_ptr(), stage.partials.numel() // 12, 0,
                 stage.exposure_grad.data_ptr(), None, None, None, 1, 0.0, 0.0, 0.0, 0.0, 0, None, st)
    return g_raw


def ctx_ps(params):
    return int(params.patch_size)


class _ImageStage:

    def __init__(self, api, exposure, alpha, exposure_grad, H, W, device):
        self.exposure = None if exposure is None else _c(exposure.detach())
        if self.exposure is not None and self.exposure.numel() != 12:
            raise ValueError("exposure: the camera's [3,4] row")
        self.alpha = None
        if alpha is not None:
            if alpha.numel() != H * W:
                raise ValueError("alpha mask of %s for a %d x %d image" % (tuple(alpha.shape), W, H))
            self.alpha = _c(alpha.detach().reshape(H, W))
        self.partials = None
        if self.exposure is not None:
            n = int(api.raw("image_stage_partials_count")(H, W))
            self.partials = torch.empty((n * 12,), dtype=torch.float32, device=device)
        if exposure_grad is not None and (exposure_grad.numel() != 12 or not exposure_grad.is_contiguous()):
            raise ValueError("exposure_grad: a contiguous [3,4] row (e.g. grad[camera] of the [n,3,4] gradient)")
        self.exposure_grad = exposure_grad
        self.raw = None


class _FusedParams:

    def __init__(self, crit, Cc, H, W):
        from .capi import GsLgdwtParams
        h1, w1 = (H + 1) // 2, (W + 1) // 2
        h2, w2 = (h1 + 1) // 2, (w1 + 1) // 2
        c = GsLgdwtParams()
        c.lambda_dssim = crit.lambda_dssim
        c.n_pix = float(Cc * H * W)
        c.n_band1, c.n_band2 = float(Cc * h1 * w1), float(Cc * h2 * w2)
        for k in range(8):
            c.dwt_w[k] = crit.dwt_weights[k]
        c.patch_w[0], c.patch_w[1] = crit.patch_lh1_weight, crit.patch_hl1_weight
        c.patch_w[2] = 0.5 * (crit.patch_lh1_weight + crit.patch_hl1_weight)
        c.patch_weight = crit.patch_dwt_weight
        hp = (crit.patch_size + 1) // 2
        c.patch_elems_per_sel = float(Cc * hp * hp)
        self.patch_enable = bool(crit.patch_dwt_enable and H >= crit.patch_size and W >= crit.patch_size)
        self.dwt_enable = bool(crit.dwt_enable)
        c.dwt_enable, c.patch_enable = int(self.dwt_enable), int(self.patch_enable)
        c.reset_sums = 1
        cb = getattr(crit, "custom_base", None)
        if cb is not None:
            c.custom_base, c.w_l1, c.w_ssim = 1, float(cb[0]), float(cb[1])
        self.clamp = bool(getattr(crit, "clamp", True))
        self.c = c
        self.patch_size = crit.patch_size
        self.n_ssim_partials = int(crit.ops.api.raw("ssim_partials_count")(1, Cc, H, W))
        self.n_dwt_partials = int(crit.ops.api.raw("dwt_partials_count")(Cc, H, W))
        self.n_l1_partials = int(crit.ops.api.raw("l1_partials_count")(Cc * H * W))
        self.fused_shape = bool(H % 4 == 0 and W % 4 == 0 and Cc <= 65535
                                and (not self.patch_enable or self.patch_size % 4 == 0))


class LGDWTCriterion:

    def __init__(self, ops, lambda_dssim=0.2, dwt_enable=True, patch_dwt_enable=True,
                 dwt_weights=(1.0, 1.0, 1.0, 0.0, 0.0, 0.0, 0.0, 0.0), patch_size=128, patch_percentile=0.2,
                 patch_dwt_weight=0.1, patch_lh1_weight=1.0, patch_hl1_weight=1.0, fused=True):
        self.ops = ops
        self.fused = fused
        self._fp = {}
        self._sums_nomask, self._no_mask = {}, {}
        self.lambda_dssim = lambda_dssim
        self.dwt_enable, self.patch_dwt_enable = dwt_enable, patch_dwt_enable
        self.dwt_weights = tuple(dwt_weights)
        self.patch_size, self.patch_percentile = patch_size, patch_percentile
        self.patch_dwt_weight = patch_dwt_weight
        self.patch_lh1_weight, self.patch_hl1_weight = patch_lh1_weight, patch_hl1_weight
        self.dwt_running_mean = None

    def elf_mask(self, gt_image):
        elf = self.ops.compute_elf_map(gt_image.unsqueeze(0))
        mask, _ = self.ops.patch_mask(elf, self.patch_size, self.patch_percentile)
        mask._gs_n_sel = mask.sum().to(torch.float32).reshape(1)
        return mask

    def sums_for(self, mask, device):
        if mask is None:
            s = self._sums_nomask.get(device)
            if s is None:
                s = self._sums_nomask[device] = torch.zeros((16,), dtype=torch.float32, device=device)
            return s
        s = getattr(mask, "_gs_sums", None)
        if s is None:
            n_sel = getattr(mask, "_gs_n_sel", None)
            if n_sel is None:
                n_sel = mask.sum().to(torch.float32).reshape(1)
            s = torch.zeros((16,), dtype=torch.float32, device=device)
# ... 65 lines not shown
```

### sparse-view-3dgs-pack_amd/gsplat_amd/trainer.py

```python
import math

import torch
import torch.distributed as dist

FIELDS = (("xyz", 3), ("features", 48), ("opacity", 1), ("scaling", 3), ("rotation", 4))
FLOATS_PER_GAUSSIAN = sum(n for _, n in FIELDS)
LRS = {"xyz": 0.00016, "f_dc": 0.0025, "f_rest": 0.0025 / 20.0, "opacity": 0.025, "scaling": 0.005, "rotation": 0.001,
       "nir_albedo": 0.00016, "nir_gain": 0.0025}
NIR_FIELD = ("nir_albedo", 1)
SHARD_UNIT = 4 * 840


def expon_lr(step, lr_init, lr_final, lr_delay_steps=0, lr_delay_mult=1.0, max_steps=1000000):
    import numpy as np
    if step < 0 or (lr_init == 0.0 and lr_final == 0.0):
        return 0.0
    if lr_delay_steps > 0:
        delay_rate = lr_delay_mult + (1 - lr_delay_mult) * np.sin(0.5 * np.pi * np.clip(step / lr_delay_steps, 0, 1))
    else:
        delay_rate = 1.0
    t = np.clip(step / max_steps, 0, 1)
    log_lerp = np.exp(np.log(lr_init) * (1 - t) + np.log(lr_final) * t)
    return float(delay_rate * log_lerp)

# ... 591 lines not shown
                view.copy_(g)
            p.grad = view

    def update_view_statistics(self, radii, viewspace_grad, into_delta=False):
        api = getattr(self.optimizer, "api", None)
        if into_delta:
            self.stat_delta.zero_()
        acc = self.stat_delta[0] if into_delta else self.xyz_gradient_accum
        den = self.stat_delta[1] if into_delta else self.denom
        if api is not None and hasattr(api, "_densify_stats") and viewspace_grad is not None and viewspace_grad.is_contiguous():
            api.call("densify_stats", radii.data_ptr(), viewspace_grad.data_ptr(), self.P, self.max_radii2D.data_ptr(),
                     acc.data_ptr(), den.data_ptr(), _stream_of(radii))
            return
        if into_delta:
            vm = (radii > 0).to(torch.float32)
            torch.maximum(self.max_radii2D, radii.to(torch.float32), out=self.max_radii2D)
            acc += torch.norm(viewspace_grad[:, :2], dim=-1) * vm
            den += vm
            return
        torch.maximum(self.max_radii2D, radii.to(torch.float32), out=self.max_radii2D)
        self.add_densification_stats(viewspace_grad, radii > 0)

    def add_densification_stats(self, viewspace_grad, visible_mask):
        vm = visible_mask.to(torch.float32).unsqueeze(-1)
        self.xyz_gradient_accum += torch.norm(viewspace_grad[:, :2], dim=-1, keepdim=True) * vm
        self.denom += vm


class _TorchAdamWithFeatureSplit:

    def __init__(self, groups, features, lr_dc, lr_rest):
        self.features = features
        self.f_dc = features.detach()[:, :1, :].clone().requires_grad_(True)
        self.f_rest = features.detach()[:, 1:, :].clone().requires_grad_(True)
        groups = groups + [{"params": [self.f_dc], "lr": lr_dc, "name": "f_dc"},
                           {"params": [self.f_rest], "lr": lr_rest, "name": "f_rest"}]
        self.opt = torch.optim.Adam(groups, lr=0.0, eps=1e-15)

    def set_xyz_lr(self, lr):
        for g in self.opt.param_groups:
            if g["name"] == "xyz":
                g["lr"] = lr

    def step(self):
        self.f_dc.grad = self.features.grad[:, :1, :].contiguous()
        self.f_rest.grad = self.features.grad[:, 1:, :].contiguous()
        self.opt.step()
        with torch.no_grad():
            self.features[:, :1, :] = self.f_dc
            self.features[:, 1:, :] = self.f_rest


def render(viewpoint_camera, pc, Rasterizer, Settings, bg_color, scaling_modifier=1.0, antialiasing=False,
           debug=False, filter_as_indices=True, clamp=True, fused=False, use_trained_exp=False, camera_index=None,
           raw_activations=False, camera_key=None):
    act = pc.fused_activations() if fused and not raw_activations else None
    if raw_activations:
        act = (pc.params["scaling"], pc.params["rotation"], pc.params["opacity"])
        screenspace_points = torch.empty_like(pc.get_xyz).requires_grad_(True)
    elif act is None:
        screenspace_points = torch.zeros_like(pc.get_xyz, dtype=pc.get_xyz.dtype, requires_grad=True) + 0
        try:
            screenspace_points.retain_grad()
        except Exception:
            pass
        act = (pc.get_scaling, pc.get_rotation, pc.get_opacity)
    else:
        screenspace_points = torch.empty_like(pc.get_xyz).requires_grad_(True)
    scales, rotations, opacities = act
    rs = Settings(
        image_height=int(viewpoint_camera.image_height), image_width=int(viewpoint_camera.image_width),
        tanfovx=math.tan(viewpoint_camera.FoVx * 0.5), tanfovy=math.tan(viewpoint_camera.FoVy * 0.5), bg=bg_color,
        scale_modifier=scaling_modifier, viewmatrix=viewpoint_camera.world_view_transform,
        projmatrix=viewpoint_camera.full_proj_transform, sh_degree=pc.active_sh_degree,
        campos=viewpoint_camera.camera_center, prefiltered=False, debug=debug, antialiasing=antialiasing)
    rasterizer = Rasterizer(raster_settings=rs)
    if camera_key is not None:
        rasterizer.camera_key = camera_key
        rasterizer.camera_limits = False
    rendered_image, radii, depth_image = rasterizer(
        means3D=pc.get_xyz, means2D=screenspace_points, shs=pc.get_features, colors_precomp=None,
        opacities=opacities, scales=scales, rotations=rotations, cov3D_precomp=None)
    if use_trained_exp:
        exposure = pc.get_exposure(camera_index)
        rendered_image = torch.matmul(rendered_image.permute(1, 2, 0), exposure[:3, :3]).permute(2, 0, 1) + \
            exposure[:3, 3, None, None]
    if clamp:
        rendered_image = rendered_image.clamp(0, 1)
    return {"render": rendered_image, "viewspace_points": screenspace_points,
            "visibility_filter": None if filter_as_indices is None else
            ((radii > 0).nonzero() if filter_as_indices else (radii > 0)),
            "radii": radii, "depth": depth_image}


def camera_to(cam, device):
    return cam._replace(world_view_transform=cam.world_view_transform.to(device),
                        full_proj_transform=cam.full_proj_transform.to(device),
                        camera_center=cam.camera_center.to(device))


class TrainOptions:

    def __init__(self, **kw):
        self.iterations = 30_000
        self.position_lr_final = 0.0000016
        self.position_lr_delay_mult = 0.01
        self.position_lr_max_steps = 30_000
        self.densification_interval = 100
        self.opacity_reset_interval = 3000
        self.densify_from_iter = 500
        self.densify_until_iter = 15_000
        self.densify_grad_threshold = 0.0002
        self.min_opacity = 0.005
        self.size_threshold = 20
        self.sh_increase_interval = 1000
        self.depth_l1_weight_init = 1.0
        self.depth_l1_weight_final = 0.01
        self.optimizer_type = "default"
        self.white_background = False
        self.random_background = False
        self.cameras_extent = 1.0
        self.seed = 0
        for k, v in kw.items():
            if not hasattr(self, k):
                raise TypeError("unknown option %s" % k)
            setattr(self, k, v)


def cameras_extent(camera_centers):
    c = torch.stack([torch.as_tensor(x, dtype=torch.float64).reshape(3) for x in camera_centers])
    return float((c - c.mean(dim=0, keepdim=True)).norm(dim=1).max() * 1.1)


class Trainer:

    def __init__(self, model, cameras, gt_images, criterion, Rasterizer, Settings, bg, rank=0, world_size=1,
                 optimizer_step=True, masks=None, sharded_optimizer=None, sparse_exchange=None, optimizer_type="default",
                 alpha_masks=None):
        import os
        self.sharded_optimizer = (os.environ.get("GS_SHARDED_ADAM", "1") == "1") if sharded_optimizer is None \
            else bool(sharded_optimizer)
        self.sparse_exchange = (os.environ.get("GS_SPARSE_EXCHANGE", "0") == "1") if sparse_exchange is None \
            else bool(sparse_exchange)
        self.last_exchange = None
        if optimizer_type not in ("default", "sparse_adam"):
            raise ValueError("optimizer_type must be 'default' or 'sparse_adam'")
        self.optimizer_type = optimizer_type
        if optimizer_type == "sparse_adam":
            if not isinstance(model.optimizer, FlatAdam):
                raise RuntimeError("sparse_adam needs the flat Adam state (a model built with an api)")
            model.optimizer.sparse = True
            self.sharded_optimizer = False
        self.model, self.cameras, self.gts, self.criterion = model, cameras, gt_images, criterion
        self.Rasterizer, self.Settings, self.bg = Rasterizer, Settings, bg
        self.rank, self.world_size = rank, world_size
        self.optimizer_step = optimizer_step
        self.masks = masks
        self.alpha_masks = alpha_masks
        self._bg_gen = None
        self.depth_priors = None
        self.depth_l1_weight = 0.0
        self.last = None
        Trainer._uids = getattr(Trainer, "_uids", 0) + 1
        self.uid = Trainer._uids
        be = getattr(getattr(getattr(self.Rasterizer, "_fn", None), "_impl", None), "backend", None)
        if be is not None and hasattr(be, "drop_camera_entries"):
            import weakref
            weakref.finalize(self, be.drop_camera_entries, ("trainer", self.uid))
        self._stack = []
        self._rng = None

    def camera_index(self, k):
        return (k * self.world_size + self.rank) % len(self.cameras)

    def step(self, k):
        return self._step_camera(self.camera_index(k), self.optimizer_step, ())

    def draw_cameras(self, seed):
        import random
        if self._rng is None:
            self._rng = random.Random(seed)
        mine = None
        for r in range(self.world_size):
            if not self._stack:
                self._stack = list(range(len(self.cameras)))
            ci = self._stack.pop(self._rng.randint(0, len(self._stack) - 1))
            if r == self.rank:
                mine = ci
        return mine

    densify_decisions = None
    alpha_masks = None
    _bg_gen = None
    _use_stage = False

    def train_iteration(self, iteration, opt):
        self.sync()
        m = self.model
        m.update_learning_rate(iteration, opt.position_lr_final, opt.position_lr_delay_mult, opt.position_lr_max_steps,
                               exposure_max_steps=opt.iterations)
        if iteration % opt.sh_increase_interval == 0:
            m.oneupSHdegree()
        if self.depth_priors is not None:
            self.depth_l1_weight = expon_lr(iteration, opt.depth_l1_weight_init, opt.depth_l1_weight_final, max_steps=opt.iterations)
        ci = self.draw_cameras(opt.seed)
        if opt.random_background:
            self._draw_background(opt.seed)
        in_densify = iteration < opt.densify_until_iter
        will_densify = in_densify and iteration > opt.densify_from_iter and iteration % opt.densification_interval == 0
        will_reset = in_densify and (iteration % opt.opacity_reset_interval == 0 or
                                     (opt.white_background and iteration == opt.densify_from_iter))
        do_step = iteration < opt.iterations and not will_densify
        loss = self._step_camera(ci, do_step, ("opacity",) if will_reset else (), exposure_step=iteration < opt.iterations)
        if will_densify or will_reset or iteration >= opt.iterations:
            self.sync()
        densified, reset = None, False
        if will_densify:
            self.gather_optimizer_state()
            thr = opt.size_threshold if iteration > opt.opacity_reset_interval else None
            gen = torch.Generator().manual_seed(opt.seed * 1000003 + iteration)
            dec = self.densify_decisions(iteration) if self.densify_decisions is not None else None
            densified = m.densify_and_prune(opt.densify_grad_threshold, opt.min_opacity, opt.cameras_extent, thr,
                                            self.last["radii"], generator=gen, decisions=dec)
        if will_reset:
            m.reset_opacity()
            reset = True
        return dict(loss=loss, densified=densified, reset=reset, P=m.P, camera=ci)

    def _draw_background(self, seed):
        if self._bg_gen is None:
            dev = self.bg.device if torch.is_tensor(self.bg) else torch.device(self.model.device)
            self._bg_gen = torch.Generator(device=dev)
            self._bg_gen.manual_seed(int(seed) + self.rank)
            self.bg = torch.empty((3,), dtype=torch.float32, device=dev)
        torch.rand((3,), out=self.bg, generator=self._bg_gen)

    def _alpha(self, ci):
        return None if self.alpha_masks is None else self.alpha_masks[ci]

    def _image_extras(self):
        return self.model.exposure is not None or self.alpha_masks is not None or self._bg_gen is not None

    def _stage_ok(self):
        from .optim import ExposureAdam
        m = self.model
        return (self.optimizer_type != "sparse_adam" and type(self)._render_view is Trainer._render_view
                and type(self)._criterion_backward is Trainer._criterion_backward
                and (m.exposure is None or isinstance(m.exposure_optimizer, ExposureAdam)))

    FUSED_STEP = __import__("os").environ.get("GS_FUSED_STEP", "1") != "0"

    def _fused_step_ok(self, backend, optimizer_step):
        m = self.model
        return (self.FUSED_STEP and optimizer_step and self.world_size == 1 and backend is not None
                and isinstance(m.optimizer, FlatAdam) and (not m.with_nir or self.RENDERS_NIR) and m.flat.is_cuda
                and hasattr(backend.api, "_backward_step") and hasattr(backend, "fused_step"))

    RENDERS_NIR = False

    def _fused_dp_ok(self, backend, optimizer_step):
        m = self.model
        return (self.FUSED_STEP and optimizer_step and self.world_size > 1 and backend is not None
                and isinstance(m.optimizer, FlatAdam) and (not m.with_nir or self.RENDERS_NIR) and m.flat.is_cuda
                and hasattr(backend.api, "_backward_step") and hasattr(backend.api, "_adam_step_gated")
                and hasattr(backend, "fused_step"))

    depth_limit = None
    RAW_ACTIVATIONS = True

    def sync(self):
        g = getattr(self, "_graphed", None)
        if g is not None:
            g.settle()
        p, self._pending = getattr(self, "_pending", None), None
        if p is None:
            return
        if "flag_host" in p:
            p["event"].synchronize()
            if p["verdict"] is not None:
                p["verdict"]()
            if float(p["flag_host"][0]) == 0.0:
                return
        elif p["verdict"]():
            return
        opt = self.model.optimizer
        opt.t, opt.seg_steps = p["counters"][0], dict(p["counters"][1])
        if p.get("exposure_steps") is not None:
            self.model.exposure_optimizer.steps = p["exposure_steps"]
        if p["running_mean"] is not None:
            self.criterion.dwt_running_mean.copy_(p["running_mean"])
        p["loss"].copy_(self._step_camera(p["ci"], True, p["skip"], exposure_step=p.get("exposure_step")))
        self.sync()

    def checkpoint(self):
        self.sync()
        self.gather_optimizer_state()
        return self.model.capture()

    def _backend(self):
        be = getattr(getattr(self.Rasterizer, "_fn", None), "_impl", None)
        return getattr(be, "backend", None)

    MANUAL_BACKWARD = __import__("os").environ.get("GS_MANUAL_BACKWARD", "1") != "0"

    class _ManualCtx:

# ... 841 lines not shown
```

Before: 1184.

## Fold LGDWT loss combine into fused forward kernel via last-block ticket

Adds a fused forward+combine kernel. Each workgroup publishes its SSIM and DWT partials with agent-scope atomic stores, then takes a ticket. The last workgroup to arrive performs the loss combine reduction and resets the ticket. This removes a separate combine kernel launch and its dependency gap per training step. In exchange it adds a global atomic per workgroup and a serial tail on one block, and it relies on memory-ordering correctness across workgroups. The Trainer enables it by default, and an env var can fall back to the split path.

Result: slower. 1123 (-5.1%).

```diff
diff --git a/include/gsplat.h b/include/gsplat.h
--- a/include/gsplat.h
+++ b/include/gsplat.h
@@ -305,6 +305,10 @@
 int gs_lgdwt_fused_fwd(const float* raw, const float* gt, int32_t C, int32_t H, int32_t W, float C1, float C2, int32_t ps,
                        const uint8_t* mask, float* dwt_partials, float* ssim_partials, float* dm_dmu1, float* dm_dsigma1_sq,
                        float* dm_dsigma12, void* stream);
+int gs_lgdwt_fused_fwd_combine(const float* raw, const float* gt, int32_t C, int32_t H, int32_t W, float C1, float C2,
+                               int32_t ps, const uint8_t* mask, float* dwt_partials, float* ssim_partials, float* dm_dmu1,
+                               float* dm_dsigma1_sq, float* dm_dsigma12, const float* sums, float* running_mean,
+                               const GsLgdwtParams* params , float* out, uint32_t* ticket, void* stream);
 int gs_lgdwt_fused_bwd(const float* raw, const float* gt, int32_t C, int32_t H, int32_t W, int32_t flags, int32_t ps,
                        const uint8_t* mask, const float* coef_dev, const float* dm_dmu1, const float* dm_dsigma1_sq,
                        const float* dm_dsigma12, float* grad, void* stream);
diff --git a/profiles/summarize.py b/profiles/summarize.py
--- a/profiles/summarize.py
+++ b/profiles/summarize.py
@@ -33,7 +33,7 @@
         "status_tag_kernel", "rs_small_sort_kernel", "step_uninstanced_kernel", "chain_kernel",
         "tb_entries_kernel", "tb_emit_kernel", "tb_regions_from_counts_kernel", "tb_regions_kernel", "tb_tile_count_kernel",
         "tb_region_scan_kernel", "tb_tile_scan_kernel", "tb_write_kernel", "depth_l1_kernel", "rows_pack_kernel", "row_mask_kernel",
-        "ssim_fwd_clamp_kernel", "lgdwt_bwd_kernel", "lgdwt_fwd_kernel")
+        "ssim_fwd_clamp_kernel", "lgdwt_bwd_kernel", "lgdwt_fwd_kernel", "lgdwt_fwd_combine_kernel")
 
 
 def short(name):
@@ -112,7 +112,8 @@
             "duplicate": "duplicate_kernel", "tile_ranges": "tile_ranges_kernel", "region_bin": "region_bin_kernel",
             "ssim_fwd": "ssim_fwd_kernel", "ssim_bwd": "ssim_bwd_kernel",
             "step_uninstanced": "step_uninstanced_kernel", "chain": "chain_kernel"}
-for st, kn in (("ssim_fwd", "ssim_fwd_clamp_kernel"), ("ssim_fwd", "lgdwt_fwd_kernel"), ("ssim_bwd", "lgdwt_bwd_kernel")):
+for st, kn in (("ssim_fwd", "ssim_fwd_clamp_kernel"), ("ssim_fwd", "lgdwt_fwd_kernel"), ("ssim_fwd", "lgdwt_fwd_combine_kernel"),
+               ("ssim_bwd", "lgdwt_bwd_kernel")):
     if kn in traffic:
         stage_of[st] = kn
 out = {st: traffic[k] for st, k in stage_of.items() if k in traffic}
diff --git a/sparse-view-3dgs-pack_amd/csrc/gs_loss.hip b/sparse-view-3dgs-pack_amd/csrc/gs_loss.hip
--- a/sparse-view-3dgs-pack_amd/csrc/gs_loss.hip
+++ b/sparse-view-3dgs-pack_amd/csrc/gs_loss.hip
@@ -198,7 +198,7 @@
   o.l2[0] = b2.ll; o.l2[1] = b2.lh; o.l2[2] = b2.hl; o.l2[3] = b2.hh;
 }
 
-template <bool FAST, bool ROWS>
+template <bool FAST, bool ROWS, bool PUBLISH = false>
 __device__ __forceinline__ void dwt2_l1_fwd_body(const float* __restrict__ pred, const float* __restrict__ gt, int C, int H,
                                                  int W, float* band_sums, float* l1_sum, float* __restrict__ clamped_out,
                                                  const uint8_t* __restrict__ patch_mask, int ps, float* patch_sums,
@@ -265,7 +265,9 @@
     if (threadIdx.x < 12) {
       float t = 0.f;
       for (int w = 0; w < GS_BLOCK / 64; w++) t += red12[w][threadIdx.x];
-      if (ROWS || partials)
+      if (PUBLISH)
+        __hip_atomic_store(&partials[(size_t)wg * 12 + threadIdx.x], t, __ATOMIC_RELAXED, __HIP_MEMORY_SCOPE_AGENT);
+      else if (ROWS || partials)
         partials[(size_t)wg * 12 + threadIdx.x] = t;
       else if (t != 0.f)
         atomicAdd(threadIdx.x < 8 ? &band_sums[threadIdx.x] : (threadIdx.x == 8 ? l1_sum : &patch_sums[threadIdx.x - 9]), t);
@@ -665,6 +667,7 @@
   }
   return msum;
 }
+template <bool PUBLISH = false>
 __device__ __forceinline__ void ssim_store_partial(float msum, float* __restrict__ partials, int linear) {
   __shared__ float red[GS_BLOCK / 64];
   float x = msum;
@@ -673,8 +676,13 @@
   __syncthreads();
   if ((threadIdx.x & 63) == 0) red[threadIdx.x >> 6] = x;
   __syncthreads();
-  if (threadIdx.x == 0)
-    partials[linear] = (red[0] + red[1]) + (red[2] + red[3]);
+  if (threadIdx.x == 0) {
+    const float t = (red[0] + red[1]) + (red[2] + red[3]);
+    if (PUBLISH)
+      __hip_atomic_store(&partials[linear], t, __ATOMIC_RELAXED, __HIP_MEMORY_SCOPE_AGENT);
+    else
+      partials[linear] = t;
+  }
 }
 
 __global__ void __launch_bounds__(GS_BLOCK) ssim_fwd_kernel(const float* __restrict__ img1, const float* __restrict__ img2,
@@ -814,6 +822,7 @@
 #define LGDWT_DWT 2
 #define LGDWT_CLAMP_MASK 4
 constexpr int SSIM_FWD_LDS_WORDS = (2 * SH * (SH + 1) > 5 * SH * HS) ? 2 * SH * (SH + 1) : 5 * SH * HS;
+template <bool PUBLISH = false>
 __device__ __forceinline__ void ssim_fwd_clamp_body(const float* __restrict__ raw, const float* __restrict__ gt, int H, int W,
                                                     int planes, float C1, float C2, float* __restrict__ dm_dmu1,
                                                     float* __restrict__ dm_dsigma1_sq, float* __restrict__ dm_dsigma12,
@@ -829,7 +838,7 @@
   float out[4][5];
   ssim_conv_tile<5, true>(tile, hor, out);
   const float msum = ssim_fwd_pixels(out, plane, H, W, bx, by, C1, C2, nullptr, dm_dmu1, dm_dsigma1_sq, dm_dsigma12);
-  ssim_store_partial(msum, partials, tl.linear);
+  ssim_store_partial<PUBLISH>(msum, partials, tl.linear);
 }
 __global__ void __launch_bounds__(GS_BLOCK) ssim_fwd_clamp_kernel(const float* __restrict__ raw, const float* __restrict__ gt,
                                                                   int H, int W, int planes, float C1, float C2,
@@ -839,14 +848,13 @@
   ssim_fwd_clamp_body(raw, gt, H, W, planes, C1, C2, dm_dmu1, dm_dsigma1_sq, dm_dsigma12, partials, blockIdx.x, lds_buf);
 }
 
-__global__ void __launch_bounds__(GS_BLOCK) lgdwt_fwd_kernel(const float* __restrict__ raw, const float* __restrict__ gt, int C,
-                                                             int H, int W, float C1, float C2,
-                                                             const uint8_t* __restrict__ patch_mask, int ps,
-                                                             float* __restrict__ dwt_partials, unsigned n_dwt, unsigned dwt_every,
-                                                             float* __restrict__ dm_dmu1, float* __restrict__ dm_dsigma1_sq,
-                                                             float* __restrict__ dm_dsigma12, float* __restrict__ ssim_partials) {
+template <bool PUBLISH, typename PARTIALS>
+__device__ __forceinline__ void lgdwt_fwd_body(const float* __restrict__ raw, const float* __restrict__ gt, int C, int H, int W,
+                                               float C1, float C2, const uint8_t* __restrict__ patch_mask, int ps,
+                                               PARTIALS dwt_partials, unsigned n_dwt, unsigned dwt_every,
+                                               float* __restrict__ dm_dmu1, float* __restrict__ dm_dsigma1_sq,
+                                               float* __restrict__ dm_dsigma12, PARTIALS ssim_partials, float* lds_buf) {
   static_assert(SSIM_FWD_LDS_WORDS >= (GS_BLOCK / 64) * 12, "red12 lives in the SSIM tile buffer");
-  __shared__ float lds_buf[SSIM_FWD_LDS_WORDS];
   const unsigned row = blockIdx.x >> 3, lane8 = blockIdx.x & 7, dwt_rows = (n_dwt + 7) >> 3;
   bool is_dwt;
   unsigned sub_row;
@@ -866,11 +874,126 @@
   const unsigned b = sub_row * 8 + lane8;
   if (is_dwt) {
     if (b >= n_dwt) return;
-    dwt2_l1_fwd_body<true, true>(raw, gt, C, H, W, dwt_partials, dwt_partials, nullptr, patch_mask, ps, dwt_partials,
-                                 dwt_partials, 1, b, n_dwt, reinterpret_cast<float (*)[12]>(lds_buf));
+    dwt2_l1_fwd_body<true, true, PUBLISH>(raw, gt, C, H, W, dwt_partials, dwt_partials, nullptr, patch_mask, ps, dwt_partials,
+                                          dwt_partials, 1, b, n_dwt, reinterpret_cast<float (*)[12]>(lds_buf));
   } else {
-    ssim_fwd_clamp_body(raw, gt, H, W, C, C1, C2, dm_dmu1, dm_dsigma1_sq, dm_dsigma12, ssim_partials, b, lds_buf);
-  }
+    ssim_fwd_clamp_body<PUBLISH>(raw, gt, H, W, C, C1, C2, dm_dmu1, dm_dsigma1_sq, dm_dsigma12, ssim_partials, b, lds_buf);
+  }
+}
+__global__ void __launch_bounds__(GS_BLOCK) lgdwt_fwd_kernel(const float* __restrict__ raw, const float* __restrict__ gt, int C,
+                                                             int H, int W, float C1, float C2,
+                                                             const uint8_t* __restrict__ patch_mask, int ps,
+                                                             float* __restrict__ dwt_partials, unsigned n_dwt, unsigned dwt_every,
+                                                             float* __restrict__ dm_dmu1, float* __restrict__ dm_dsigma1_sq,
+                                                             float* __restrict__ dm_dsigma12, float* __restrict__ ssim_partials) {
+  __shared__ float lds_buf[SSIM_FWD_LDS_WORDS];
+  lgdwt_fwd_body<false, float* __restrict__>(raw, gt, C, H, W, C1, C2, patch_mask, ps, dwt_partials, n_dwt, dwt_every, dm_dmu1,
+                                             dm_dsigma1_sq, dm_dsigma12, ssim_partials, lds_buf);
+}
+
+template <int NT>
+__device__ __forceinline__ void lgdwt_combine_body(const float* sums_in, float* running_mean, const GsLgdwtParams& p, float* out,
+                                                   float* ssim_partials, int n_partials, float* dwt_partials, int n_dwt,
+                                                   float* l1_partials, int n_l1, float* s_extra, float* red) {
+  static_assert(NT % 64 == 0 && 1024 % NT == 0, "whole waves that divide the 16 virtual ones evenly");
+  const int lane = threadIdx.x & 63;
+  for (int vw = threadIdx.x >> 6; vw < 16; vw += NT / 64) {
+    if (vw < 13) {
+      float t = 0.f;
+      if (vw < 12) {
+        for (int w = lane; w < n_dwt; w += 64) t += dwt_partials[(size_t)w * 12 + vw];
+      } else {
+        for (int w = lane; w < n_l1; w += 64) t += l1_partials[w];
+      }
+#pragma unroll
+      for (int off = 32; off >= 1; off >>= 1) t += __shfl_down(t, off, 64);
+      if (lane == 0) s_extra[vw] = t;
+    }
+    float part = 0.f;
+    for (int i = vw * 64 + lane; i < n_partials; i += 1024) part += ssim_partials[i];
+#pragma unroll
+    for (int off = 32; off >= 1; off >>= 1) part += __shfl_down(part, off, 64);
+    if (lane == 0) red[vw] = part;
+  }
+  __syncthreads();
+  if (threadIdx.x != 0) return;
+  float sums[16];
+#pragma unroll
+  for (int k = 0; k < 16; k++) sums[k] = sums_in[k];
+  sums[0] += s_extra[8] + s_extra[12];
+#pragma unroll
+  for (int k = 0; k < 8; k++) sums[2 + k] += s_extra[k];
+#pragma unroll
+  for (int k = 0; k < 3; k++) sums[10 + k] += s_extra[9 + k];
+  const float l1 = sums[0] / p.n_pix;
+  float ptot = 0.f;
+  for (int w = 0; w < 16; w++) ptot += red[w];
+  const float ssim = (sums[1] + ptot) / p.n_pix;
+  const float w_l1 = p.custom_base ? p.w_l1 : 1.0f - p.lambda_dssim, w_ssim = p.custom_base ? p.w_ssim : p.lambda_dssim;
+  const float base = w_l1 * l1 + w_ssim * (1.0f - ssim);
+  float loss = base;
+  float dwt = 0.f, scale = 0.f, patch = 0.f;
+  for (int k = 0; k < 24; k++) out[k] = 0.f;
+  out[7] = running_mean[0];
+  if (p.dwt_enable) {
+    for (int k = 0; k < 8; k++) {
+      const float cnt = k < 4 ? p.n_band1 : p.n_band2;
+      dwt += p.dwt_w[k] * (sums[2 + k] / cnt);
+    }
+    const float ratio = base / (dwt + 1e-8f);
+    const float m = 0.95f * running_mean[0] + 0.05f * ratio;
+    running_mean[0] = m;
+    scale = fminf(fmaxf(m, 0.1f), 10.0f);
+    loss = base + scale * dwt;
+    for (int k = 0; k < 8; k++) out[10 + k] = scale * p.dwt_w[k] / (k < 4 ? p.n_band1 : p.n_band2);
+  }
+  if (p.patch_enable) {
+    const float denom = fmaxf(sums[13] * p.patch_elems_per_sel, 1.0f);
+    for (int k = 0; k < 3; k++) {
+      patch += p.patch_w[k] * (sums[10 + k] / denom);
+      out[18 + k] = p.patch_weight * p.patch_w[k] / denom;
+    }
+    loss = loss + p.patch_weight * patch;
+  }
+  out[0] = loss; out[1] = base; out[2] = dwt; out[3] = patch; out[4] = scale; out[5] = l1; out[6] = ssim;
+  out[8] = w_l1 / p.n_pix;
+  out[9] = -w_ssim / p.n_pix;
+  if (p.reset_sums) {
+    float* z = const_cast<float*>(sums_in);
+    for (int k = 0; k < 13; k++) z[k] = 0.f;
+  }
+}
+
+__global__ void __launch_bounds__(GS_BLOCK) lgdwt_fwd_combine_kernel(const float* __restrict__ raw, const float* __restrict__ gt,
+                                                                     int C, int H, int W, float C1, float C2,
+                                                                     const uint8_t* __restrict__ patch_mask, int ps,
+                                                                     float* dwt_partials, unsigned n_dwt, unsigned dwt_every,
+                                                                     float* __restrict__ dm_dmu1, float* __restrict__ dm_dsigma1_sq,
+                                                                     float* __restrict__ dm_dsigma12, float* ssim_partials,
+                                                                     int n_partials, const float* sums_in, float* running_mean,
+                                                                     GsLgdwtParams p, float* out, unsigned* ticket) {
+  static_assert(SSIM_FWD_LDS_WORDS >= 64, "the tail's words live in the SSIM tile buffer");
+  __shared__ float lds_buf[SSIM_FWD_LDS_WORDS];
+  lgdwt_fwd_body<true, float*>(raw, gt, C, H, W, C1, C2, patch_mask, ps, dwt_partials, n_dwt, dwt_every, dm_dmu1, dm_dsigma1_sq,
+                               dm_dsigma12, ssim_partials, lds_buf);
+  asm volatile("s_waitcnt vmcnt(0)" ::: "memory");
+  __syncthreads();
+  unsigned* flag = reinterpret_cast<unsigned*>(lds_buf);
+  if (threadIdx.x == 0) {
+    const unsigned t = __hip_atomic_fetch_add(ticket, 1u, __ATOMIC_RELAXED, __HIP_MEMORY_SCOPE_AGENT);
+    const bool last = t == gridDim.x - 1;
+    if (last) {
+      __builtin_amdgcn_fence(__ATOMIC_ACQUIRE, "agent");
+      asm volatile("s_waitcnt vmcnt(0)" ::: "memory");
+    }
+    flag[0] = last ? 1u : 0u;
+  }
+  __syncthreads();
+  if (flag[0] == 0u) return;
+  lgdwt_combine_body<GS_BLOCK>(sums_in, running_mean, p, out, ssim_partials, n_partials, dwt_partials, (int)n_dwt, nullptr, 0,
+                               lds_buf + 16, lds_buf + 32);
+  if (threadIdx.x == 0)
+    __hip_atomic_store(ticket, 0u, __ATOMIC_RELAXED, __HIP_MEMORY_SCOPE_AGENT);
 }
 
 __device__ __forceinline__ void dwt2_l1_adjoint_col(const float (&a)[4], const float (&b)[4], int c4, const float (&cf)[8],
@@ -1302,78 +1425,9 @@
                                                              const float* __restrict__ dwt_partials, int n_dwt,
                                                              const float* __restrict__ l1_partials, int n_l1) {
   __shared__ float s_extra[13];
-  {
-    const int slot = threadIdx.x >> 6, lane = threadIdx.x & 63;
-    if (slot < 13) {
-      float t = 0.f;
-      if (slot < 12) {
-        for (int w = lane; w < n_dwt; w += 64) t += dwt_partials[(size_t)w * 12 + slot];
-      } else {
-        for (int w = lane; w < n_l1; w += 64) t += l1_partials[w];
-      }
-#pragma unroll
-      for (int off = 32; off >= 1; off >>= 1) t += __shfl_down(t, off, 64);
-      if (lane == 0) s_extra[slot] = t;
-    }
-  }
-  __syncthreads();
-  float sums[16];
-#pragma unroll
-  for (int k = 0; k < 16; k++) sums[k] = 0.f;
-  if (threadIdx.x == 0) {
-#pragma unroll
-    for (int k = 0; k < 16; k++) sums[k] = sums_in[k];
-    sums[0] += s_extra[8] + s_extra[12];
-#pragma unroll
-    for (int k = 0; k < 8; k++) sums[2 + k] += s_extra[k];
-#pragma unroll
-    for (int k = 0; k < 3; k++) sums[10 + k] += s_extra[9 + k];
-  }
   __shared__ float red[16];
-  float part = 0.f;
-  for (int i = threadIdx.x; i < n_partials; i += 1024) part += ssim_partials[i];
-#pragma unroll
-  for (int off = 32; off >= 1; off >>= 1) part += __shfl_down(part, off, 64);
-  if ((threadIdx.x & 63) == 0) red[threadIdx.x >> 6] = part;
-  __syncthreads();
-  if (threadIdx.x != 0) return;
-  const float l1 = sums[0] / p.n_pix;
-  float ptot = 0.f;
-  for (int w = 0; w < 16; w++) ptot += red[w];
-  const float ssim = (sums[1] + ptot) / p.n_pix;
-  const float w_l1 = p.custom_base ? p.w_l1 : 1.0f - p.lambda_dssim, w_ssim = p.custom_base ? p.w_ssim : p.lambda_dssim;
-  const float base = w_l1 * l1 + w_ssim * (1.0f - ssim);
-  float loss = base;
-  float dwt = 0.f, scale = 0.f, patch = 0.f;
-  for (int k = 0; k < 24; k++) out[k] = 0.f;
-  out[7] = running_mean[0];
-  if (p.dwt_enable) {
-    for (int k = 0; k < 8; k++) {
-      const float cnt = k < 4 ? p.n_band1 : p.n_band2;
-      dwt += p.dwt_w[k] * (sums[2 + k] / cnt);
-    }
-    const float ratio = base / (dwt + 1e-8f);
-    const float m = 0.95f * running_mean[0] + 0.05f * ratio;
-    running_mean[0] = m;
-    scale = fminf(fmaxf(m, 0.1f), 10.0f);
-    loss = base + scale * dwt;
-    for (int k = 0; k < 8; k++) out[10 + k] = scale * p.dwt_w[k] / (k < 4 ? p.n_band1 : p.n_band2);
-  }
-  if (p.patch_enable) {
-    const float denom = fmaxf(sums[13] * p.patch_elems_per_sel, 1.0f);
-    for (int k = 0; k < 3; k++) {
-      patch += p.patch_w[k] * (sums[10 + k] / denom);
-      out[18 + k] = p.patch_weight * p.patch_w[k] / denom;
-    }
-    loss = loss + p.patch_weight * patch;
-  }
-  out[0] = loss; out[1] = base; out[2] = dwt; out[3] = patch; out[4] = scale; out[5] = l1; out[6] = ssim;
-  out[8] = w_l1 / p.n_pix;
-  out[9] = -w_ssim / p.n_pix;
-  if (p.reset_sums) {
-    float* z = const_cast<float*>(sums_in);
-    for (int k = 0; k < 13; k++) z[k] = 0.f;
-  }
+  lgdwt_combine_body<1024>(sums_in, running_mean, p, out, const_cast<float*>(ssim_partials), n_partials,
+                           const_cast<float*>(dwt_partials), n_dwt, const_cast<float*>(l1_partials), n_l1, s_extra, red);
 }
 
 int gs_lgdwt_combine_pp(const float* sums, const float* ssim_partials, int64_t n_partials, const float* dwt_partials,
@@ -1442,6 +1496,39 @@
   GS_LAUNCH_CHECK(s, 0);
   return GS_OK;
 }
+int gs_lgdwt_fused_fwd_combine(const float* raw, const float* gt, int32_t C, int32_t H, int32_t W, float C1, float C2, int32_t ps,
+                               const uint8_t* mask, float* dwt_partials, float* ssim_partials, float* dm_dmu1,
+                               float* dm_dsigma1_sq, float* dm_dsigma12, const float* sums, float* running_mean,
+                               const GsLgdwtParams* p, float* out, uint32_t* ticket, void* stream) {
+  if (!raw || !gt || !dwt_partials || !ssim_partials || !dm_dmu1 || !dm_dsigma1_sq || !dm_dsigma12) return GS_E_NULL;
+  if (!sums || !running_mean || !p || !out || !ticket) return GS_E_NULL;
+  const int rc = lgdwt_fused_args(C, H, W, ps, mask);
+  if (rc != GS_OK) return rc;
+  if (!lgdwt_fused_ok(raw, gt, dm_dmu1, dm_dsigma1_sq, dm_dsigma12, C, H, W)) return GS_E_UNSUPPORTED;
+  const int64_t n_partials = gs_ssim_partials_count(1, C, H, W);
+  if (n_partials > 0x7FFFFFFF) return GS_E_SHAPE;
+  static const bool split = [] {
+    const char *a = getenv("GS_LGDWT_COMBINE_SPLIT"), *b = getenv("GS_LGDWT_FWD_SPLIT");
+    return (a && atoi(a) != 0) || (b && atoi(b) != 0);
+  }();
+  if (split) {
+    const int r = gs_lgdwt_fused_fwd(raw, gt, C, H, W, C1, C2, ps, mask, dwt_partials, ssim_partials, dm_dmu1, dm_dsigma1_sq,
+                                     dm_dsigma12, stream);
+    if (r != GS_OK) return r;
+    return gs_lgdwt_combine_pp(sums, ssim_partials, n_partials, dwt_partials, gs_dwt_partials_count(C, H, W), nullptr, 0,
+                               running_mean, p, out, stream);
+  }
+  hipStream_t s = (hipStream_t)stream;
+  const unsigned n_ssim = ssim_launch_blocks(W, H, C), n_dwt = dwt2_fwd_workgroups(C, H, W);
+  const unsigned ssim_rows = n_ssim / 8, dwt_rows = (n_dwt + 7) / 8;
+  const unsigned every = ssim_rows / dwt_rows < 4 ? ssim_rows / dwt_rows : 4;
+  GS_PROF(ST_SSIM_FWD, s);
+  hipLaunchKernelGGL(lgdwt_fwd_combine_kernel, dim3((ssim_rows + dwt_rows) * 8), dim3(GS_BLOCK), 0, s, raw, gt, C, H, W, C1, C2,
+                     mask, ps, dwt_partials, n_dwt, every, dm_dmu1, dm_dsigma1_sq, dm_dsigma12, ssim_partials, (int)n_partials,
+                     sums, running_mean, *p, out, (unsigned*)ticket);
+  GS_LAUNCH_CHECK(s, 0);
+  return GS_OK;
+}
 int gs_lgdwt_fused_bwd(const float* raw, const float* gt, int32_t C, int32_t H, int32_t W, int32_t flags, int32_t ps,
                        const uint8_t* mask, const float* coef_dev, const float* dm_dmu1, const float* dm_dsigma1_sq,
                        const float* dm_dsigma12, float* grad, void* stream) {
diff --git a/sparse-view-3dgs-pack_amd/gsplat_amd/capi.py b/sparse-view-3dgs-pack_amd/gsplat_amd/capi.py
--- a/sparse-view-3dgs-pack_amd/gsplat_amd/capi.py
+++ b/sparse-view-3dgs-pack_amd/gsplat_amd/capi.py
@@ -185,6 +185,8 @@
     "ssim_partials_count": (C.c_int64, [_I32, _I32, _I32, _I32]),
     "ssim_fwd_partials": (C.c_int, [_P, _P, _I32, _I32, _I32, _I32, _F, _F, _P, _P, _P, _P, _P]),
     "lgdwt_fused_fwd": (C.c_int, [_P, _P, _I32, _I32, _I32, _F, _F, _I32, _P, _P, _P, _P, _P, _P, _P]),
+    "lgdwt_fused_fwd_combine": (C.c_int, [_P, _P, _I32, _I32, _I32, _F, _F, _I32, _P, _P, _P, _P, _P, _P, _P, _P,
+                                          C.POINTER(GsLgdwtParams), _P, _P, _P]),
     "lgdwt_fused_bwd": (C.c_int, [_P, _P, _I32, _I32, _I32, _I32, _I32, _P, _P, _P, _P, _P, _P, _P]),
     "adam_step": (C.c_int, [_P, _P, _P, _P, _I64, C.POINTER(GsAdamSeg), _I32, _F, _F, _F, _I32, _P]),
     "adam_step_gated": (C.c_int, [_P, _P, _P, _P, _I64, C.POINTER(GsAdamSeg), _I32, _F, _F, _F, _I32, _P, _P]),
@@ -210,7 +212,7 @@
 DEVICE_ONLY = ("export_row_mask", "backward_step", "backward_step_x", "step_uninstanced", "export_tile_order", "export_tile_stop_depth", "forward_status", "forward_bin", "export_binning_region", "debug_blend_stats", "adam_step_gated", "tile_depth_limit_floats", "profile_enable", "profile_only", "profile_reset", "profile_stage_count", "profile_stage_name", "profile_read",
                "forward_render_x", "backward_x", "forward_tile_order",
                "image_stage_partials_count", "image_stage_fwd", "image_stage_bwd", "exposure_adam",
-               "lgdwt_fused_fwd", "lgdwt_fused_bwd",
+               "lgdwt_fused_fwd", "lgdwt_fused_bwd", "lgdwt_fused_fwd_combine",
                "grid_encode_tmp_bytes", "grid_encode_fwd", "grid_encode_bwd", "sh_encode_fwd", "sh_encode_bwd")
 
 ERRORS = {-1: "GS_E_NULL", -2: "GS_E_SHAPE", -3: "GS_E_SCRATCH", -4: "GS_E_OVERFLOW", -5: "GS_E_UNSUPPORTED"}
diff --git a/sparse-view-3dgs-pack_amd/gsplat_amd/losses.py b/sparse-view-3dgs-pack_amd/gsplat_amd/losses.py
--- a/sparse-view-3dgs-pack_amd/gsplat_amd/losses.py
+++ b/sparse-view-3dgs-pack_amd/gsplat_amd/losses.py
@@ -24,6 +24,8 @@
     def __init__(self, api):
         self.api = api
         self._unit = {}
+        self._tickets = {}
+        self.fold_combine = False
         ops = self
 
         class _L1(torch.autograd.Function):
@@ -187,6 +189,14 @@
             u = self._unit[device] = torch.ones((), dtype=torch.float32, device=device)
         return u
 
+    def combine_ticket(self, device):
+        device = torch.device(device)
+        key = (device, torch.cuda.current_stream(device).cuda_stream)
+        t = self._tickets.get(key)
+        if t is None:
+            t = self._tickets[key] = torch.zeros((1,), dtype=torch.int32, device=device)
+        return t
+
     def l1_loss(self, network_output, gt):
         return self._L1.apply(network_output, gt)
 
@@ -279,6 +289,7 @@
         patch_folded = bool(params.patch_enable and params.dwt_enable and H % 4 == 0 and W % 4 == 0
                             and ctx_ps(params) % 4 == 0)
         dwt_part = l1_part = None
+        out = None
         fast = H % 4 == 0 and W % 4 == 0
         fused = bool(FUSED_PASSES and params.fused_shape and hasattr(api, "_lgdwt_fused_bwd")
                      and (patch_folded or not params.patch_enable) and raw.data_ptr() % 16 == 0 and gt.data_ptr() % 16 == 0)
@@ -289,9 +300,15 @@
         if fused and (patch_folded or (params.dwt_enable and params.clamp)):
             img = None
             dwt_part = torch.empty((params.n_dwt_partials * 12,), dtype=torch.float32, device=raw.device)
-            api.call("lgdwt_fused_fwd", raw.data_ptr(), gt.data_ptr(), Cc, H, W, 0.01 ** 2, 0.03 ** 2,
-                     ctx_ps(params) if patch_folded else 0, mask.data_ptr() if patch_folded else None, dwt_part.data_ptr(),
-                     partials.data_ptr(), d1.data_ptr(), d2.data_ptr(), d3.data_ptr(), st)
+            fwd_args = (raw.data_ptr(), gt.data_ptr(), Cc, H, W, 0.01 ** 2, 0.03 ** 2,
+                        ctx_ps(params) if patch_folded else 0, mask.data_ptr() if patch_folded else None, dwt_part.data_ptr(),
+                        partials.data_ptr(), d1.data_ptr(), d2.data_ptr(), d3.data_ptr())
+            if getattr(ops, "fold_combine", False) and hasattr(api, "_lgdwt_fused_fwd_combine"):
+                out = torch.empty((24,), dtype=torch.float32, device=raw.device)
+                api.call("lgdwt_fused_fwd_combine", *fwd_args, sums.data_ptr(), running_mean.data_ptr(), C.byref(params.c),
+                         out.data_ptr(), ops.combine_ticket(raw.device).data_ptr(), st)
+            else:
+                api.call("lgdwt_fused_fwd", *fwd_args, st)
         elif patch_folded or (params.dwt_enable and fast and params.clamp):
             img = torch.empty_like(raw)
             dwt_part = torch.empty((params.n_dwt_partials * 12,), dtype=torch.float32, device=raw.device)
@@ -313,11 +330,12 @@
         if params.patch_enable and not patch_folded:
             api.call("patch_dwt_fwd", img.data_ptr(), gt.data_ptr(), Cc, H, W, ctx_ps(params), mask.data_ptr(),
                      sums[10:].data_ptr(), st)
-        out = torch.empty((24,), dtype=torch.float32, device=raw.device)
-        api.call("lgdwt_combine_pp", sums.data_ptr(), partials.data_ptr(), partials.numel(),
-                 None if dwt_part is None else dwt_part.data_ptr(), 0 if dwt_part is None else dwt_part.numel() // 12,
-                 None if l1_part is None else l1_part.data_ptr(), 0 if l1_part is None else l1_part.numel(),
-                 running_mean.data_ptr(), C.byref(params.c), out.data_ptr(), st)
+        if out is None:
+            out = torch.empty((24,), dtype=torch.float32, device=raw.device)
+            api.call("lgdwt_combine_pp", sums.data_ptr(), partials.data_ptr(), partials.numel(),
+                     None if dwt_part is None else dwt_part.data_ptr(), 0 if dwt_part is None else dwt_part.numel() // 12,
+                     None if l1_part is None else l1_part.data_ptr(), 0 if l1_part is None else l1_part.numel(),
+                     running_mean.data_ptr(), C.byref(params.c), out.data_ptr(), st)
         ctx.ops, ctx.params, ctx.patch_folded, ctx.stage = ops, params, patch_folded, stage
         ctx.save_for_backward(raw, img, gt, mask, d1, d2, d3, out)
         ctx.mark_non_differentiable(out)
diff --git a/sparse-view-3dgs-pack_amd/gsplat_amd/trainer.py b/sparse-view-3dgs-pack_amd/gsplat_amd/trainer.py
--- a/sparse-view-3dgs-pack_amd/gsplat_amd/trainer.py
+++ b/sparse-view-3dgs-pack_amd/gsplat_amd/trainer.py
@@ -767,6 +767,8 @@
             model.optimizer.sparse = True
             self.sharded_optimizer = False
         self.model, self.cameras, self.gts, self.criterion = model, cameras, gt_images, criterion
+        if getattr(criterion, "ops", None) is not None:
+            criterion.ops.fold_combine = True
         self.Rasterizer, self.Settings, self.bg = Rasterizer, Settings, bg
         self.rank, self.world_size = rank, world_size
         self.optimizer_step = optimizer_step
```
